# Rayhane-mamah/Tacotron-2

Hardware: NVIDIA H100
Metric: wavenet_train_audio_samples_per_sec (higher is better)
Workload: dtype bf16

## Files before the change

include/t2b200.h:

```cpp
#ifndef T2B200_H_
#define T2B200_H_

#include <stdint.h>

#ifdef __cplusplus
extern "C" {
#endif

#define T2B200_ABI_VERSION 3

#define T2_OK 0
#define T2_ERR_INVALID_ARG (-1)
#define T2_ERR_UNSUPPORTED_SHAPE (-2)
#define T2_ERR_CUDA (-3)
#define T2_ERR_NCCL (-4)

const char* t2_last_error(void);
int t2_abi_version(void);
int t2_struct_size(const char* name);
long long t2_launch_count(void);

int t2_dbg_conv_gemm(const void* d_a, int B, int T, int C, int ld, const int* shifts, int nshift,
                     const void* d_w, int N, int BN, const float* d_bias, int relu, void* d_out_bf16,
                     float* d_out_f32, void* stream);
int t2_dbg_set_timing_buffer(long long* d_buf);
int t2_dbg_wgrad(const void* d_a, int Ca, const void* d_bm, int Cb, int B, int T, int shift_a, float scale,
                 float* d_out, void* stream);

typedef struct {
  const void* ptr;
  int C, T, B, L, ld;
} t2_dbg_act_t;
typedef struct {
  int map, shift, k0, nkb, layer0, nlayers;
} t2_dbg_seg_t;
typedef struct {
  t2_dbg_act_t a[4];
  int na;
  t2_dbg_seg_t seg[16];
  int nseg;
  const void* w;
  int wN, wK, wL, w_layer, w_k0;
  int T, B, n_tiles, ksplit, epi, BN;
  int cluster;
  int cluster_used;
  void* ptr[12];
  float f[6];
  int i[12];
  unsigned long long seed;
} t2_dbg_gemm_t;
int t2_dbg_act_gemm(t2_dbg_gemm_t* call, void* stream);
typedef struct {
  int a_map, a_ch0, a_shift, a_layer;
  int b_map, b_ch0, b_shift, b_layer;
  long long out_off;
  int ldc, m_valid, n_valid;
  float scale;
  int accumulate;
  const float* div;
} t2_dbg_wgrad_tile_t;
int t2_dbg_wgrad_tiles(const t2_dbg_act_t* maps, int nmaps, const t2_dbg_wgrad_tile_t* tiles, int ntiles, float* d_out, int T, int B,
                       void* stream);
int t2_dbg_fx_colsum(const float* d_addends, int nrows, int ncols, float* d_out, void* stream);

typedef struct {
  int kernel;
  void* p[16];
  long long i[16];
  float f[4];
  unsigned long long seed;
  const unsigned long long* step;
} t2_dbg_kernel_t;
#define T2_DBG_TACO_ATT_FWD 1
#define T2_DBG_TACO_BN_FWD 2
#define T2_DBG_TACO_BN_BWD 3
#define T2_DBG_TACO_CELL_BWD 4
#define T2_DBG_TACO_ATT_FINISH 5
#define T2_DBG_TACO_DVALUES 6
#define T2_DBG_TACO_ATT_BWD 7
#define T2_DBG_TACO_CONV_GEMM 8
#define T2_DBG_TACO_LSTM_STEP 9
#define T2_DBG_TACO_ROWS 10
int t2_dbg_taco_kernel(const t2_dbg_kernel_t* call, void* stream);
#define T2_DBG_CBHG_BN_FWD 1
#define T2_DBG_CBHG_BN_BWD 2
#define T2_DBG_CBHG_POOL_FWD 3
#define T2_DBG_CBHG_POOL_BWD 4
#define T2_DBG_CBHG_HIGHWAY_FWD 5
#define T2_DBG_CBHG_HIGHWAY_BWD 6
#define T2_DBG_CBHG_GRU_FWD 7
#define T2_DBG_CBHG_GRU_BWD 8
int t2_dbg_cbhg_kernel(const t2_dbg_kernel_t* call, void* stream);


typedef struct {
  int layers, stacks, residual_channels, gate_channels, skip_out_channels;
  int kernel_size;
  int cin_channels;
  int out_channels;
  int quantize_channels;
  int input_type;
  int legacy, residual_legacy;
  int upsample_type;
  int n_upsample;
  int upsample_scales[4];
  int freq_axis_kernel_size;
  float dropout;
  float log_scale_min;
  int B, T, Tc;
  int c_pre_upsampled;
  float log_scale_min_gauss;
  int cdf_loss;
  int split_bf16;
  int gin_channels;
  int n_speakers;
  int upsample_activation;
  float leaky_alpha;
} t2_wn_config_t;

typedef struct {
  long long n_params;
  long long packed_bytes;
  long long workspace_bytes;
  int n_tensors;
} t2_wn_sizes_t;

int t2_wn_sizes(const t2_wn_config_t* cfg, t2_wn_sizes_t* out);
int t2_wn_param_info(const t2_wn_config_t* cfg, int i, char* name, int name_cap, long long* offset, int* ndim,
                     int* shape4);
int t2_wn_init(const t2_wn_config_t* cfg, void* d_packed, void* d_workspace, void* stream);
int t2_wn_pack_weights(const t2_wn_config_t* cfg, const float* d_params, void* d_packed, void* d_workspace,
                       void* stream);
int t2_wn_forward(const t2_wn_config_t* cfg, const float* d_params, const void* d_packed, void* d_workspace,
                  const void* d_x, const float* d_c, const void* d_targets, const int* d_lengths, float* d_loss,
                  float* d_logits, int save_for_backward, unsigned long long seed,
                  const unsigned long long* d_step, void* stream);
int t2_wn_backward(const t2_wn_config_t* cfg, const float* d_params, const void* d_packed, void* d_workspace,
                   const void* d_x, const float* d_c, float* d_grads, unsigned long long seed,
                   const unsigned long long* d_step, void* stream);
int t2_wn_backward_phased(const t2_wn_config_t* cfg, const float* d_params, const void* d_packed, void* d_workspace,
                          const void* d_x, const float* d_c, float* d_grads, unsigned long long seed,
                          const unsigned long long* d_step, int phase, int n_groups, void* stream);
int t2_wn_time_kernel(const t2_wn_config_t* cfg, const float* d_params, const void* d_packed, void* d_workspace,
                      int which, int layer, int reps, float* ms_per_launch, void* stream);
int t2_dbg_wn_per_layer(int mode);
int t2_dbg_wn_chain(const t2_wn_config_t* cfg, int dir, int* out, int cap);
int t2_wn_workspace_tensor(const t2_wn_config_t* cfg, void* d_workspace, const char* name, void** ptr,
                           long long* count, int* elem_bytes);
int t2_wn_set_speakers(const t2_wn_config_t* cfg, void* d_workspace, const int* d_speaker_ids, void* stream);
#define T2_DBG_WN_UP_FWD 1
#define T2_DBG_WN_UP_BWD_PARAM 2
#define T2_DBG_WN_UP_BWD_INPUT 3
#define T2_DBG_WN_FIRST_CONV 10
#define T2_DBG_WN_FIRST_CONV_BWD 11
#define T2_DBG_WN_COLSUM 12
#define T2_DBG_WN_DERIVED_BIAS 13
#define T2_DBG_WN_SKIP_BIAS 14
#define T2_DBG_WN_FX_FINALIZE 15
#define T2_DBG_WN_CL_TO_CHW 16
#define T2_DBG_WN_GIN_BIAS 17
#define T2_DBG_WN_SET_SPEAKERS 18
#define T2_DBG_WN_GIN_WGRAD 19
#define T2_DBG_WN_GIN_DEMB 20
int t2_dbg_wn_kernel(const t2_dbg_kernel_t* call, void* stream);


int t2_wn_ar_sizes(const t2_wn_config_t* cfg, int cluster_size, long long* packed_bytes, long long* workspace_bytes);
int t2_wn_ar_pack(const t2_wn_config_t* cfg, int cluster_size, const float* d_params, void* d_packed_ar,
                  void* d_workspace, void* stream);
int t2_wn_ar_generate(const t2_wn_config_t* cfg, int cluster_size, const float* d_params, const void* d_packed_ar,
                      void* d_workspace, const float* d_c, const void* d_initial, const void* d_test_inputs,
                      const float* d_u_a, const float* d_u_b, unsigned long long seed, void* d_out_samples,
                      float* d_out_raw, void* stream);
int t2_wn_ar_set_speakers(const t2_wn_config_t* cfg, int cluster_size, const float* d_params, const void* d_packed_ar,
                          void* d_workspace, const int* d_speaker_ids, void* stream);


typedef struct {
  int B, T_in, T_out;
  int n_symbols, num_mels, embedding_dim;
  int enc_conv_layers, enc_conv_kernel, enc_conv_channels, encoder_lstm_units;
  int attention_dim, attention_filters, attention_kernel;
  int prenet1, prenet2, decoder_lstm_units;
  int postnet_layers, postnet_kernel, postnet_channels;
  int clip_outputs;
  float dropout_rate;
  float zoneout_rate;
  float reg_weight;
  float max_abs_value, lower_bound_decay;
  int split_bf16;
  int mask_decoder;
  float cross_entropy_pos_weight;
  int unmasked_encoder;
  int noncumulative_weights;
  float teacher_forcing_ratio;
} t2_taco_config_t;

int t2_taco_sizes(const t2_taco_config_t* cfg, long long* n_params, long long* packed_bytes, long long* workspace_bytes,
                  int* n_tensors);
int t2_taco_param_info(const t2_taco_config_t* cfg, int i, char* name, int name_cap, long long* offset, int* ndim,
                       int* shape4, int* trainable);
int t2_taco_init(const t2_taco_config_t* cfg, void* d_packed, void* d_workspace, void* stream);
int t2_taco_pack_weights(const t2_taco_config_t* cfg, const float* d_params, void* d_packed, void* d_workspace, void* stream);
int t2_taco_forward(const t2_taco_config_t* cfg, float* d_params, const void* d_packed, void* d_workspace,
                    const int* d_inputs, const int* d_input_lengths, const float* d_mel_targets,
                    const float* d_stop_targets, float* d_loss, int training, unsigned long long seed,
                    const unsigned long long* d_step, void* stream);
int t2_taco_set_target_lengths(const t2_taco_config_t* cfg, void* d_workspace, const int* d_target_lengths, void* stream);
int t2_taco_backward(const t2_taco_config_t* cfg, const float* d_params, const void* d_packed, void* d_workspace,
                     const int* d_inputs, const int* d_input_lengths, const float* d_mel_targets,
                     const float* d_stop_targets, float* d_grads, unsigned long long seed,
                     const unsigned long long* d_step, void* stream);
int t2_taco_backward_ex(const t2_taco_config_t* cfg, const float* d_params, const void* d_packed, void* d_workspace,
                     const int* d_inputs, const int* d_input_lengths, const float* d_mel_targets,
                     const float* d_stop_targets, float* d_grads, const float* d_mel_outputs_grad, unsigned long long seed,
                     const unsigned long long* d_step, void* stream);
int t2_taco_infer_begin(const t2_taco_config_t* cfg, float* d_params, const void* d_packed, void* d_workspace,
                        const int* d_inputs, const int* d_input_lengths, void* stream);
int t2_taco_infer_steps(const t2_taco_config_t* cfg, float* d_params, const void* d_packed, void* d_workspace,
                        const int* d_input_lengths, int t_begin, int t_end, unsigned long long seed, void* stream);
int t2_taco_infer_finish(const t2_taco_config_t* cfg, float* d_params, const void* d_packed, void* d_workspace, int T_used,
                         void* stream);
int t2_rng_uniform_f32(unsigned long long seed, unsigned int stream_id, long long first_index, long long n, float* d_out,
                       void* stream);
int t2_dbg_att_stamps(long long* d_buf);
int t2_dbg_ar_stamps(long long* d_buf);
int t2_taco_workspace_tensor(const t2_taco_config_t* cfg, void* d_workspace, const char* name, void** ptr,
                             long long* count, int* elem_bytes);

typedef struct {
  int B, T;
  int num_mels;
  int kernels;
  int conv_channels;
  int pool_size;
  int projection;
  int projection_kernel_size;
  int highwaynet_layers;
  int highway_units;
  int rnn_units;
  int num_freq;
  int n_priority_freq;
  int clip_outputs, mask_decoder;
  float max_abs_value, lower_bound_decay, reg_weight;
  int split_bf16;
} t2_cbhg_config_t;
int t2_cbhg_sizes(const t2_cbhg_config_t* cfg, long long* n_params, long long* packed_bytes, long long* workspace_bytes, int* n_tensors);
int t2_cbhg_param_info(const t2_cbhg_config_t* cfg, int i, char* name, int name_cap, long long* offset, int* ndim, int* shape4,
                       int* trainable);
int t2_cbhg_init(const t2_cbhg_config_t* cfg, void* d_packed, void* d_workspace, void* stream);
int t2_cbhg_pack_weights(const t2_cbhg_config_t* cfg, const float* d_params, void* d_packed, void* d_workspace, void* stream);
int t2_cbhg_set_target_lengths(const t2_cbhg_config_t* cfg, void* d_workspace, const int* d_target_lengths, void* stream);
int t2_cbhg_forward(const t2_cbhg_config_t* cfg, float* d_params, const void* d_packed, void* d_workspace, const float* d_mel,
                    const float* d_linear_targets, float* d_loss, int training, void* stream);
int t2_cbhg_backward(const t2_cbhg_config_t* cfg, const float* d_params, const void* d_packed, void* d_workspace, const float* d_mel,
                     float* d_grads, float* d_mel_grad, void* stream);
int t2_cbhg_workspace_tensor(const t2_cbhg_config_t* cfg, void* d_workspace, const char* name, void** ptr, long long* count);

int t2_adam_step(float* d_params, const float* d_grads, float* d_m, float* d_v, float* d_ema,
                 const long long* d_offsets, int n_tensors, long long n_total, float lr, float beta1, float beta2,
                 float eps, int step, float grad_scale, float max_norm, float max_value, float global_norm_clip,
                 float ema_decay, float* d_scratch, void* stream);

typedef struct {
  int sample_rate, n_fft, hop_size, win_size, num_mels;
  float fmin, fmax;
  float magnitude_power;
  float min_level_db, ref_level_db, max_abs_value;
  int symmetric_mels, allow_clipping_in_normalization, signal_normalization;
} t2_audio_config_t;

int t2_stft_mel_plan_bytes(const t2_audio_config_t* cfg, long long* bytes);
int t2_stft_mel_plan_init(const t2_audio_config_t* cfg, void* d_plan, void* stream);
int t2_stft_mel_frames(const t2_audio_config_t* cfg, int n_samples);
int t2_stft_mel_f32(const t2_audio_config_t* cfg, const void* d_plan, const float* d_wav, int B, int n_samples,
                    float preemphasis, float gain, float* d_mel, float* d_linear, int time_major, void* stream);
int t2_mel_basis_f64(const t2_audio_config_t* cfg, double* h_basis);
int t2_griffin_lim_bytes(const t2_audio_config_t* cfg, int B, int frames, long long* bytes);
int t2_griffin_lim_f32(const t2_audio_config_t* cfg, const void* d_plan, const float* d_mag, float* d_phase_io, int B, int frames,
                       int iters, unsigned long long seed, void* d_workspace, float* d_wav, void* stream);
int t2_preemphasis_f32(const float* d_x, float* d_y, int B, int n_samples, float k, void* stream);
int t2_mulaw_quantize_f32_i32(const float* d_in, int* d_out, long long n, void* stream);
int t2_inv_mulaw_quantize_i32_f32(const int* d_in, float* d_out, long long n, void* stream);
int t2_mulaw_f32(const float* d_in, float* d_out, long long n, void* stream);
int t2_inv_mulaw_f32(const float* d_in, float* d_out, long long n, void* stream);

#ifdef __cplusplus
}
#endif
#endif
```

tacotron-2_b200/csrc/t2_api.cu:

```cuda
#include <stdarg.h>
#include <stdio.h>
#include <stddef.h>
#include <string.h>

#include <vector>

#include "../../include/t2b200.h"
#include "t2_common.cuh"
#include "t2_gemm.h"

#include <atomic>
static thread_local char g_err[512] = "";
static std::atomic<long long> g_launches{0};
void t2_count_launch(int n) { g_launches.fetch_add(n, std::memory_order_relaxed); }
extern "C" long long t2_launch_count(void) { return g_launches.load(std::memory_order_relaxed); }

int t2_set_error(int code, const char* fmt, ...) {
  va_list ap;
  va_start(ap, fmt);
  vsnprintf(g_err, sizeof(g_err), fmt, ap);
  va_end(ap);
  return code;
}

extern "C" const char* t2_last_error(void) { return g_err; }
extern "C" int t2_abi_version(void) { return T2B200_ABI_VERSION; }

extern "C" int t2_dbg_conv_gemm(const void* a, int B, int T, int C, int ld, const int* shifts, int nshift,
                                const void* w, int N, int BN, const float* bias, int relu, void* out_bf16,
                                float* out_f32, void* stream) {
  using namespace t2;
  T2_REQUIRE(nshift >= 1 && nshift <= kMaxSeg, T2_ERR_INVALID_ARG, "nshift out of range");
  T2_REQUIRE(BN == 128 || BN == 256, T2_ERR_UNSUPPORTED_SHAPE, "BN must be 128 or 256");
  ActGemmCall c;
  memset(&c, 0, sizeof(c));
  c.a[0] = make_act(a, C, T, B, 1, ld);
  c.na = 1;
  const int nkb = (C + kBK - 1) / kBK;
  for (int s = 0; s < nshift; ++s) c.seg[s] = Seg{0, shifts[s], 0, nkb, 0, 1};
  c.nseg = nshift;
  c.w = w; c.wN = N; c.wK = nshift * nkb * kBK; c.wL = 1; c.w_layer = 0;
  c.T = T; c.B = B; c.n_tiles = (N + BN - 1) / BN;
  c.epi.ptr[0] = out_bf16; c.epi.ptr[1] = const_cast<float*>(bias); c.epi.ptr[2] = out_f32;
  c.epi.i[0] = N; c.epi.i[1] = relu; c.epi.i[2] = N;
  return launch_act_gemm(EPI_BIAS_ACT, BN, c, static_cast<cudaStream_t>(stream));
}

extern "C" int t2_dbg_wgrad(const void* a, int Ca, const void* bm, int Cb, int B, int T, int shift_a,
                            float scale, float* out, void* stream) {
  using namespace t2;
  ActT maps[2] = {make_act(a, Ca, T, B), make_act(bm, Cb, T, B)};
  WgradTile proto;
  memset(&proto, 0, sizeof(proto));
  proto.a_map = 0; proto.a_shift = shift_a; proto.b_map = 1; proto.scale = scale;
  std::vector<WgradTile> tiles;
  append_wgrad_tiles(tiles, proto, 0, Ca, 0, Cb, 0, Cb);
  WgradTile* dt = nullptr;
  cudaStream_t st = static_cast<cudaStream_t>(stream);
  T2_CHECK_CUDA(cudaMallocAsync(&dt, tiles.size() * sizeof(WgradTile), st));
  T2_CHECK_CUDA(cudaMemcpyAsync(dt, tiles.data(), tiles.size() * sizeof(WgradTile), cudaMemcpyHostToDevice, st));
  int rc = launch_wgrad(maps, 2, dt, int(tiles.size()), out, T, B, st);
  cudaStreamSynchronize(st);
  cudaFreeAsync(dt, st);
  return rc;
}

#define T2_SAME_FIELD(A, B, f) static_assert(offsetof(A, f) == offsetof(B, f), #A " / " #B ": field " #f)
static_assert(sizeof(t2_dbg_act_t) == sizeof(t2::ActT), "t2_dbg_act_t / ActT");
T2_SAME_FIELD(t2_dbg_act_t, t2::ActT, ptr); T2_SAME_FIELD(t2_dbg_act_t, t2::ActT, C); T2_SAME_FIELD(t2_dbg_act_t, t2::ActT, ld);
static_assert(sizeof(t2_dbg_seg_t) == sizeof(t2::Seg), "t2_dbg_seg_t / Seg");
T2_SAME_FIELD(t2_dbg_seg_t, t2::Seg, map); T2_SAME_FIELD(t2_dbg_seg_t, t2::Seg, nlayers);
static_assert(sizeof(t2_dbg_wgrad_tile_t) == sizeof(t2::WgradTile), "t2_dbg_wgrad_tile_t / WgradTile");
T2_SAME_FIELD(t2_dbg_wgrad_tile_t, t2::WgradTile, a_map); T2_SAME_FIELD(t2_dbg_wgrad_tile_t, t2::WgradTile, a_ch0);
T2_SAME_FIELD(t2_dbg_wgrad_tile_t, t2::WgradTile, a_shift); T2_SAME_FIELD(t2_dbg_wgrad_tile_t, t2::WgradTile, a_layer);
T2_SAME_FIELD(t2_dbg_wgrad_tile_t, t2::WgradTile, b_map); T2_SAME_FIELD(t2_dbg_wgrad_tile_t, t2::WgradTile, b_ch0);
T2_SAME_FIELD(t2_dbg_wgrad_tile_t, t2::WgradTile, b_shift); T2_SAME_FIELD(t2_dbg_wgrad_tile_t, t2::WgradTile, b_layer);
T2_SAME_FIELD(t2_dbg_wgrad_tile_t, t2::WgradTile, out_off); T2_SAME_FIELD(t2_dbg_wgrad_tile_t, t2::WgradTile, ldc);
T2_SAME_FIELD(t2_dbg_wgrad_tile_t, t2::WgradTile, m_valid); T2_SAME_FIELD(t2_dbg_wgrad_tile_t, t2::WgradTile, n_valid);
T2_SAME_FIELD(t2_dbg_wgrad_tile_t, t2::WgradTile, scale); T2_SAME_FIELD(t2_dbg_wgrad_tile_t, t2::WgradTile, accumulate);
T2_SAME_FIELD(t2_dbg_wgrad_tile_t, t2::WgradTile, div);
#undef T2_SAME_FIELD

extern "C" int t2_dbg_act_gemm(t2_dbg_gemm_t* call, void* stream) {
  using namespace t2;
  T2_REQUIRE(call != nullptr, T2_ERR_INVALID_ARG, "null call");
  T2_REQUIRE(call->na >= 1 && call->na <= 4 && call->nseg >= 1 && call->nseg <= kMaxSeg, T2_ERR_INVALID_ARG,
             "bad map/segment count (%d, %d)", call->na, call->nseg);
  ActGemmCall c;
  memset(&c, 0, sizeof(c));
  memcpy(c.a, call->a, sizeof(c.a));
  c.na = call->na;
  memcpy(c.seg, call->seg, sizeof(c.seg));
  c.nseg = call->nseg;
  c.w = call->w; c.wN = call->wN; c.wK = call->wK; c.wL = call->wL; c.w_layer = call->w_layer; c.w_k0 = call->w_k0;
  c.T = call->T; c.B = call->B; c.n_tiles = call->n_tiles; c.ksplit = call->ksplit; c.cluster = call->cluster;
  memcpy(c.epi.ptr, call->ptr, sizeof(c.epi.ptr));
  memcpy(c.epi.f, call->f, sizeof(c.epi.f));
  memcpy(c.epi.i, call->i, sizeof(c.epi.i));
  c.epi.seed = call->seed;
  call->cluster_used = 0;
  return launch_act_gemm(call->epi, call->BN, c, static_cast<cudaStream_t>(stream), &call->cluster_used);
}

extern "C" int t2_dbg_wgrad_tiles(const t2_dbg_act_t* maps, int nmaps, const t2_dbg_wgrad_tile_t* tiles, int ntiles, float* d_out, int T,
                                  int B, void* stream) {
  using namespace t2;
  T2_REQUIRE(maps && tiles && nmaps >= 1 && nmaps <= 6 && ntiles >= 1, T2_ERR_INVALID_ARG, "wgrad_tiles: bad map/tile arguments");
  for (int i = 0; i < ntiles; ++i)
    T2_REQUIRE(tiles[i].a_map >= 0 && tiles[i].a_map < nmaps && tiles[i].b_map >= 0 && tiles[i].b_map < nmaps &&
               tiles[i].m_valid >= 1 && tiles[i].m_valid <= 128 && tiles[i].n_valid >= 1 && tiles[i].n_valid <= 256 &&
               tiles[i].accumulate >= 0 && tiles[i].accumulate <= 2,
               T2_ERR_INVALID_ARG, "wgrad_tiles: bad tile %d", i);
  WgradTile* dt = nullptr;
  cudaStream_t st = static_cast<cudaStream_t>(stream);
  T2_CHECK_CUDA(cudaMallocAsync(&dt, ntiles * sizeof(WgradTile), st));
  const cudaError_t e = cudaMemcpyAsync(dt, tiles, ntiles * sizeof(WgradTile), cudaMemcpyHostToDevice, st);
  int rc = e == cudaSuccess ? launch_wgrad(reinterpret_cast<const ActT*>(maps), nmaps, dt, ntiles, d_out, T, B, st)
                            : t2_set_error(T2_ERR_CUDA, "wgrad_tiles: tile table upload failed: %s", cudaGetErrorString(e));
  cudaStreamSynchronize(st);
  cudaFreeAsync(dt, st);
  return rc;
}

__global__ void fx_colsum_kernel(const float* __restrict__ v, long long n, int ncols, long long* acc) {
  const long long i = blockIdx.x * (long long)blockDim.x + threadIdx.x;
  if (i < n) t2::fx_add(acc + i % ncols, v[i]);
}
extern "C" int t2_dbg_fx_colsum(const float* d_addends, int nrows, int ncols, float* d_out, void* stream) {
  T2_REQUIRE(d_addends && d_out && nrows >= 0 && ncols >= 1, T2_ERR_INVALID_ARG, "fx_colsum: bad arguments");
  cudaStream_t st = static_cast<cudaStream_t>(stream);
  long long* acc = nullptr;
  T2_CHECK_CUDA(cudaMallocAsync(&acc, size_t(ncols) * sizeof(long long), st));
  const long long n = (long long)nrows * ncols;
  cudaError_t e = cudaMemsetAsync(acc, 0, size_t(ncols) * sizeof(long long), st);
  if (e == cudaSuccess) e = cudaMemsetAsync(d_out, 0, size_t(ncols) * sizeof(float), st);
  if (e == cudaSuccess && n > 0) {
    fx_colsum_kernel<<<unsigned((n + 255) / 256), 256, 0, st>>>(d_addends, n, ncols, acc);
    t2_count_launch();
    e = cudaGetLastError();
  }
  int rc = e == cudaSuccess ? t2::launch_fx_finalize(acc, d_out, ncols, st)
                            : t2_set_error(T2_ERR_CUDA, "fx_colsum: %s", cudaGetErrorString(e));
  cudaStreamSynchronize(st);
  cudaFreeAsync(acc, st);
  return rc;
}

extern "C" int t2_dbg_set_timing_buffer(long long* d_buf) {
  t2::set_timing_buffer(d_buf);
  return T2_OK;
}

__global__ void rng_uniform_kernel(unsigned long long seed, unsigned int stream, long long i0, long long n, float* __restrict__ out) {
  const long long i = blockIdx.x * (long long)blockDim.x + threadIdx.x;
  if (i < n) out[i] = t2::hash_uniform32(t2::hash_seed(seed, stream), (unsigned long long)(i0 + i));
}
extern "C" int t2_rng_uniform_f32(unsigned long long seed, unsigned int stream_id, long long first_index, long long n, float* d_out,
                                  void* stream) {
  T2_REQUIRE(n >= 0 && (n == 0 || d_out != nullptr), T2_ERR_INVALID_ARG, "rng_uniform: bad arguments");
  if (n == 0) return T2_OK;
  rng_uniform_kernel<<<unsigned((n + 255) / 256), 256, 0, static_cast<cudaStream_t>(stream)>>>(seed, stream_id, first_index, n, d_out);
  t2_count_launch();
  T2_CHECK_CUDA(cudaGetLastError());
  return T2_OK;
}

extern "C" int t2_struct_size(const char* name) {
  if (!name) return -1;
  if (!strcmp(name, "t2_wn_config_t")) return int(sizeof(t2_wn_config_t));
  if (!strcmp(name, "t2_wn_sizes_t")) return int(sizeof(t2_wn_sizes_t));
  if (!strcmp(name, "t2_taco_config_t")) return int(sizeof(t2_taco_config_t));
  if (!strcmp(name, "t2_cbhg_config_t")) return int(sizeof(t2_cbhg_config_t));
  if (!strcmp(name, "t2_audio_config_t")) return int(sizeof(t2_audio_config_t));
  if (!strcmp(name, "t2_dbg_act_t")) return int(sizeof(t2_dbg_act_t));
  if (!strcmp(name, "t2_dbg_gemm_t")) return int(sizeof(t2_dbg_gemm_t));
  if (!strcmp(name, "t2_dbg_wgrad_tile_t")) return int(sizeof(t2_dbg_wgrad_tile_t));
  if (!strcmp(name, "t2_dbg_kernel_t")) return int(sizeof(t2_dbg_kernel_t));
  return -1;
}
```

tacotron-2_b200/csrc/t2_cbhg.cu:

```cuda
#include <math.h>
#include <stdio.h>
#include <string.h>

#include <string>
#include <vector>

#include "../../include/t2b200.h"
#include "t2_batchnorm.h"
#include "t2_common.cuh"
#include "t2_gemm.h"
#include "t2_params.h"

namespace t2 {
namespace {

typedef __nv_bfloat16 bf16;
constexpr int kMaxBank = 16, kMaxHw = 8;
constexpr int kGruItems = 4;
constexpr int kGruThreads = 256;

struct CConv {
  int cin, cout, k, act;
  ConvBnParams p;
  int cinp, coutp;
// ... 493 lines not shown
      for (int q = 0; q < 2; ++q) {
        const float2 v = *reinterpret_cast<const float2*>(dcp + (2 * half + q) * kRU + 2 * jp);
        drh[q] += v.x * w0 + v.y * w1;
      }
    }
#pragma unroll
    for (int q = 0; q < 2; ++q) {
      const int i = 2 * half + q;
      const long long row = (long long)(b0 + i) * a.T + t;
      const float drp = drh[q] * hp[q] * rv[q] * (1.f - rv[q]);
      const float dup = du[q] * uv[q] * (1.f - uv[q]);
      dgp[i * 2 * kRU + k2] = drp; dgp[i * 2 * kRU + kRU + k2] = dup;
      if (b0 + i < a.B) {
        a.dXP[row * XPW + d * 3 * kRU + k2] = __float2bfloat16(drp);
        a.dXP[row * XPW + d * 3 * kRU + kRU + k2] = __float2bfloat16(dup);
      }
      part[q] += drh[q] * rv[q];
    }
    __syncthreads();
#pragma unroll 4
    for (int jp = 0; jp < 128; ++jp) {
      const uint32_t w = WgT[jp * 128 + k2];
      const float w0 = bf16lo(w), w1 = bf16hi(w);
#pragma unroll
      for (int q = 0; q < 2; ++q) {
        const float2 v = *reinterpret_cast<const float2*>(dgp + (2 * half + q) * 2 * kRU + 2 * jp);
        part[q] += v.x * w0 + v.y * w1;
      }
    }
#pragma unroll
    for (int q = 0; q < 2; ++q) dh[(2 * half + q) * kRU + k2] = part[q];
    __syncthreads();
  }
}

int gemm(const void* a, int C, int ld, int k0, long long T, int Bn, const void* w, int wN, int wK, int ntaps, const int* shifts, int BN,
         const float* bias, int act, void* out_bf16, float* out_f32, int ldo, int nvalid, cudaStream_t st, const int* k0s = nullptr, int Ctot = 0,
         int split = 0) {
  ActGemmCall g;
  memset(&g, 0, sizeof(g));
  if (split) {
    const int rc = set_split_operand(g, a, C, int(T), Bn, ntaps, shifts);
    if (rc) return rc;
  } else {
    const int nkb = (C + kBK - 1) / kBK;
    g.a[0] = make_act(a, Ctot > 0 ? Ctot : k0 + C, int(T), Bn, 1, ld); g.na = 1;
    T2_REQUIRE(ntaps <= kMaxSeg, T2_ERR_UNSUPPORTED_SHAPE, "CBHG gemm: too many taps");
    for (int s = 0; s < ntaps; ++s) g.seg[s] = Seg{0, shifts ? shifts[s] : 0, k0s ? k0s[s] : k0, nkb, 0, 1};
    g.nseg = ntaps;
  }
  g.w = w; g.wN = wN; g.wK = wK; g.wL = 1;
  g.T = int(T); g.B = Bn; g.n_tiles = (nvalid + BN - 1) / BN;
  g.epi.ptr[0] = out_bf16; g.epi.ptr[1] = const_cast<float*>(bias); g.epi.ptr[2] = out_f32;
  g.epi.i[0] = ldo; g.epi.i[1] = act; g.epi.i[2] = nvalid;
  return launch_act_gemm(EPI_BIAS_ACT, BN, g, st);
}

enum { WG_LIN = 0, WG_GRU = 1, WG_HW0 = 2  };
void build_tiles(const CL& lo, std::vector<std::vector<WgradTile>>& L) {
  L.clear();
  const int RU = lo.RU, HU = lo.HU;
  { std::vector<WgradTile> w; append_wgrad_tiles(w, dense_proto(0, 1), 0, 2 * RU, 0, lo.NF, lo.p_lk, lo.NF); L.push_back(w); }
  { std::vector<WgradTile> w;
    for (int d = 0; d < 2; ++d) {
      append_wgrad_tiles(w, dense_proto(0, 1), 0, HU, d * 3 * RU, 2 * RU, lo.p_gk[d], 2 * RU);
      append_wgrad_tiles(w, dense_proto(0, 1), 0, HU, d * 3 * RU + 2 * RU, RU, lo.p_ck[d], RU);
      append_wgrad_tiles(w, dense_proto(2, 1, d == 0 ? -1 : 1), d * RU, RU, d * 3 * RU, 2 * RU, lo.p_gk[d] + (long long)HU * 2 * RU, 2 * RU);
      append_wgrad_tiles(w, dense_proto(3 + d, 1), 0, RU, d * 3 * RU + 2 * RU, RU, lo.p_ck[d] + (long long)HU * RU, RU);
    }
    L.push_back(w); }
  for (int i = lo.NH - 1; i >= 0; --i) {
    std::vector<WgradTile> w;
    append_wgrad_tiles(w, dense_proto(0, 1), 0, HU, 0, HU, lo.p_hk[i][0], HU);
    append_wgrad_tiles(w, dense_proto(0, 1), 0, HU, HU, HU, lo.p_hk[i][1], HU);
    L.push_back(w);
  }
  { std::vector<WgradTile> w; append_wgrad_tiles(w, dense_proto(0, 1), 0, lo.M, 0, HU, lo.p_dk, HU); L.push_back(w); }
  for (const CConv* c : {&lo.proj2, &lo.proj1}) {
    std::vector<WgradTile> w; append_conv_wgrad_tiles(w, c->k, 0, c->cin, 0, c->cout, c->p.kernel); L.push_back(w);
  }
  { std::vector<WgradTile> w;
    for (int k = 1; k <= lo.K; ++k) append_conv_wgrad_tiles(w, k, 0, lo.M, (k - 1) * lo.CC, lo.CC, lo.bank[k - 1].p.kernel);
    L.push_back(w); }
}

size_t gru_fwd_smem(int split) { return (64 * 256 + 64 * 128) * 4 * (split ? 2 : 1) + 3 * kGruItems * kRU * 4; }
size_t gru_bwd_smem() { return (128 * 128 + 64 * 128) * 4 + (2 * kGruItems * kRU + kGruItems * 2 * kRU) * 4; }

int gru_setup() {
  T2_CHECK_CUDA(cudaFuncSetAttribute(gru_fwd_kernel<false>, cudaFuncAttributeMaxDynamicSharedMemorySize, int(gru_fwd_smem(0))));
  T2_CHECK_CUDA(cudaFuncSetAttribute(gru_fwd_kernel<true>, cudaFuncAttributeMaxDynamicSharedMemorySize, int(gru_fwd_smem(1))));
  T2_CHECK_CUDA(cudaFuncSetAttribute(gru_bwd_kernel, cudaFuncAttributeMaxDynamicSharedMemorySize, int(gru_bwd_smem())));
  return T2_OK;
}
int check_gru_shape(int B, int T, int HU, int RU, const char* what) {
  T2_REQUIRE(B >= 1 && T >= 1 && HU >= 1, T2_ERR_UNSUPPORTED_SHAPE, "%s: B >= 1, T >= 1, HU >= 1 (B %d, T %d, HU %d)", what, B, T, HU);
  T2_REQUIRE(RU == kRU, T2_ERR_UNSUPPORTED_SHAPE, "%s: RU must be %d (got %d)", what, kRU, RU);
  return T2_OK;
}
int check_gru_fwd(const GruArgs& a, int split) {
  T2_REQUIRE(a.params && a.XP && a.out, T2_ERR_INVALID_ARG, "gru_fwd: null params / XP / out");
  T2_REQUIRE(split == 0 || split == 1, T2_ERR_INVALID_ARG, "gru_fwd: split %d is not 0 or 1", split);
  int n = 0;
  for (int d = 0; d < 2; ++d) n += (a.r[d] != nullptr) + (a.u[d] != nullptr) + (a.c[d] != nullptr) + (a.rh[d] != nullptr);
  T2_REQUIRE(!split || n == 0, T2_ERR_INVALID_ARG, "gru_fwd: the split mode writes no stashes (%d of 8 given)", n);
  T2_REQUIRE(n == 0 || n == 8, T2_ERR_INVALID_ARG, "gru_fwd: the r / u / c / rh stashes of both directions are all present or all null (%d of 8)", n);
  for (int d = 0; d < 2; ++d)
    T2_REQUIRE(a.p_gk[d] >= 0 && a.p_ck[d] >= 0 && a.p_gb[d] >= 0 && a.p_cb[d] >= 0, T2_ERR_INVALID_ARG, "gru_fwd: negative parameter offset");
  return check_gru_shape(a.B, a.T, a.HU, a.RU, "gru_fwd");
}
int check_gru_bwd(const GruBwdArgs& a) {
  T2_REQUIRE(a.params && a.dout && a.out && a.dXP, T2_ERR_INVALID_ARG, "gru_bwd: null params / dout / out / dXP");
  for (int d = 0; d < 2; ++d) {
    T2_REQUIRE(a.r[d] && a.u[d] && a.c[d], T2_ERR_INVALID_ARG, "gru_bwd: null stash of direction %d", d);
    T2_REQUIRE(a.p_gk[d] >= 0 && a.p_ck[d] >= 0, T2_ERR_INVALID_ARG, "gru_bwd: negative parameter offset");
  }
  return check_gru_shape(a.B, a.T, a.HU, a.RU, "gru_bwd");
}
int launch_gru_fwd(const GruArgs& a, int split, cudaStream_t st) {
  int rc = check_gru_fwd(a, split);
  if (rc) return rc;
  (split ? gru_fwd_kernel<true> : gru_fwd_kernel<false>)<<<dim3((a.B + kGruItems - 1) / kGruItems, 2), kGruThreads, gru_fwd_smem(split), st>>>(a);
  t2_count_launch();
  T2_CHECK_CUDA(cudaGetLastError());
  return T2_OK;
}
int launch_gru_bwd(const GruBwdArgs& a, cudaStream_t st) {
  int rc = check_gru_bwd(a);
  if (rc) return rc;
  gru_bwd_kernel<<<dim3((a.B + kGruItems - 1) / kGruItems, 2), kGruThreads, gru_bwd_smem(), st>>>(a); t2_count_launch();
  T2_CHECK_CUDA(cudaGetLastError());
  return T2_OK;
}

}
}

using namespace t2;

extern "C" int t2_cbhg_sizes(const t2_cbhg_config_t* cfg, long long* n_params, long long* packed_bytes, long long* workspace_bytes, int* n_tensors) {
  CL lo;
  int rc = build(cfg, lo, nullptr);
  if (rc) return rc;
  if (n_params) *n_params = lo.n_params;
  if (packed_bytes) *packed_bytes = lo.packed_bytes;
  if (workspace_bytes) *workspace_bytes = lo.workspace_bytes;
  if (n_tensors) *n_tensors = int(lo.params.size());
  return T2_OK;
}

extern "C" int t2_cbhg_param_info(const t2_cbhg_config_t* cfg, int i, char* name, int cap, long long* offset, int* ndim, int* shape4, int* trainable) {
  CL lo;
  int rc = build(cfg, lo, nullptr);
  if (rc) return rc;
  return param_info(lo.params, i, name, cap, offset, ndim, shape4, trainable);
}

extern "C" int t2_cbhg_init(const t2_cbhg_config_t* cfg, void* d_packed, void* d_workspace, void* stream) {
  CL lo;
  std::vector<PackJob> jobs;
  int rc = build(cfg, lo, &jobs);
  if (rc) return rc;
  T2_REQUIRE(d_packed && d_workspace, T2_ERR_INVALID_ARG, "cbhg_init: null buffers");
  cudaStream_t st = static_cast<cudaStream_t>(stream);
  uint8_t* ws = static_cast<uint8_t*>(d_workspace);
  T2_CHECK_CUDA(cudaMemsetAsync(d_packed, 0, lo.packed_bytes, st));
  T2_CHECK_CUDA(cudaMemsetAsync(d_workspace, 0, lo.workspace_bytes, st));
  T2_CHECK_CUDA(cudaMemcpyAsync(ws + lo.w_jobs, jobs.data(), jobs.size() * sizeof(PackJob), cudaMemcpyHostToDevice, st));
  std::vector<std::vector<WgradTile>> wl;
  build_tiles(lo, wl);
  std::vector<WgradTile> all;
  for (auto& w : wl) all.insert(all.end(), w.begin(), w.end());
  T2_REQUIRE(all.size() <= 4096, T2_ERR_UNSUPPORTED_SHAPE, "cbhg: too many wgrad tiles (%d)", int(all.size()));
  T2_CHECK_CUDA(cudaMemcpyAsync(ws + lo.w_tiles, all.data(), all.size() * sizeof(WgradTile), cudaMemcpyHostToDevice, st));
  rc = upload_reg_table(lo.params, ws + lo.w_regtab, st);
  if (rc) return rc;
  rc = gru_setup();
  if (rc) return rc;
  T2_CHECK_CUDA(cudaStreamSynchronize(st));
  return T2_OK;
}

extern "C" int t2_cbhg_pack_weights(const t2_cbhg_config_t* cfg, const float* d_params, void* d_packed, void* d_workspace, void* stream) {
  CL lo;
  int rc = build(cfg, lo, nullptr);
  if (rc) return rc;
  return launch_pack(d_params, d_packed, reinterpret_cast<const PackJob*>(static_cast<uint8_t*>(d_workspace) + lo.w_jobs), lo.n_jobs, 32, 32,
                     static_cast<cudaStream_t>(stream));
}

extern "C" int t2_cbhg_set_target_lengths(const t2_cbhg_config_t* cfg, void* d_workspace, const int* d_target_lengths, void* stream) {
  CL lo;
  int rc = build(cfg, lo, nullptr);
  if (rc) return rc;
  T2_REQUIRE(d_workspace && d_target_lengths, T2_ERR_INVALID_ARG, "cbhg_set_target_lengths: null pointer");
  T2_CHECK_CUDA(cudaMemcpyAsync(static_cast<uint8_t*>(d_workspace) + lo.w_tlen, d_target_lengths, lo.B * sizeof(int), cudaMemcpyDeviceToDevice,
                                static_cast<cudaStream_t>(stream)));
  return T2_OK;
}

namespace {
struct Ctx { const CL* lo; uint8_t* ws; const uint8_t* pk; float* params; cudaStream_t st; int training; };
template <typename T> T* W(const Ctx& s, long long off) { return reinterpret_cast<T*>(s.ws + off); }

int conv_fwd(const Ctx& s, const CConv& L, const void* x, int ld_x, bf16* y_b, float* y_f, int ldo) {
  int shifts[16];
  for (int j = 0; j < L.k; ++j) shifts[j] = conv_tap_shift(L.k, j);
  const int BN = L.cout % 256 == 0 ? 256 : 128;
  const int sp = s.lo->c.split_bf16;
  return gemm(x, L.cin, ld_x, 0, s.lo->T, s.lo->B, s.pk + L.k_w, (L.cout + 127) / 128 * 128, L.k * L.cinp * (sp ? 3 : 1), L.k, shifts, BN,
              s.params + L.p.bias, L.act, y_b, y_f, ldo, L.cout, s.st, nullptr, 0, sp);
}
}

extern "C" int t2_cbhg_forward(const t2_cbhg_config_t* cfg, float* d_params, const void* d_packed, void* d_workspace, const float* d_mel,
                               const float* d_linear_targets, float* d_loss, int training, void* stream) {
  CL lo;
  int rc = build(cfg, lo, nullptr);
  if (rc) return rc;
  T2_REQUIRE(d_params && d_packed && d_workspace && d_mel, T2_ERR_INVALID_ARG, "cbhg_forward: null pointer");
  cudaStream_t st = static_cast<cudaStream_t>(stream);
  Ctx s{&lo, static_cast<uint8_t*>(d_workspace), static_cast<const uint8_t*>(d_packed), d_params, st, training};
  const long long N = lo.N;
  const int T = lo.T, B = lo.B, M = lo.M, HU = lo.HU, RU = lo.RU, KC = lo.KC, PJc = lo.PJc;
  float* scal = W<float>(s, lo.w_scal);
  T2_CHECK_CUDA(cudaMemsetAsync(scal, 0, 16 * sizeof(float), st));
  const int sp = lo.c.split_bf16, k3 = sp ? 3 : 1, Ms = (M + 63) / 64 * 64;
  bf16* x0 = W<bf16>(s, lo.w_x0);
  if (sp) launch_f32_to_bf16_split(d_mel, x0, N, M, Ms, st);
  else launch_f32_to_bf16(d_mel, x0, N * M, st);
  bf16* Y = W<bf16>(s, lo.w_Y);
  float* Yf = W<float>(s, lo.w_Y);
  bf16* Xb = W<bf16>(s, lo.w_Xb);
  float* stb = W<float>(s, lo.w_stb);
  if (training) T2_CHECK_CUDA(cudaMemsetAsync(stb, 0, 2LL * KC * sizeof(float), st));
  for (int k = 1; k <= lo.K; ++k) {
    const CConv& L = lo.bank[k - 1];
    const int c0 = (k - 1) * lo.CC;
// ... 331 lines not shown
```

tacotron-2_b200/csrc/t2_common.cuh:

```cuda
#pragma once
#include <cuda.h>
#include <cuda_bf16.h>
#include <cuda_runtime.h>
#include <stdint.h>

#define T2_OK 0
#define T2_ERR_INVALID_ARG (-1)
#define T2_ERR_UNSUPPORTED_SHAPE (-2)
#define T2_ERR_CUDA (-3)
#define T2_ERR_NCCL (-4)

int t2_set_error(int code, const char* fmt, ...);
void t2_count_launch(int n = 1);
#define T2_CHECK_CUDA(expr)                                                              \
  do {                                                                                   \
    cudaError_t _e = (expr);                                                             \
    if (_e != cudaSuccess)                                                               \
      return t2_set_error(T2_ERR_CUDA, "%s:%d %s -> %s", __FILE__, __LINE__, #expr,      \
                          cudaGetErrorString(_e));                                       \
  } while (0)
#define T2_REQUIRE(cond, code, ...)                                                      \
  do {                                                                                   \
    if (!(cond)) return t2_set_error(code, __VA_ARGS__);                                 \
  } while (0)
// ... 103 lines not shown
  if (fx_in_range(v)) {
    x.a = v;
    x.old = static_cast<long long>(atomicAdd(x.d, static_cast<unsigned long long>(v)));
  }
  return x;
}
__device__ __forceinline__ void fx_check(const FxAdd& x) {
  if (!fx_in_range(x.old) || !fx_in_range(x.old + x.a)) atomicExch(x.d, static_cast<unsigned long long>(kFxPoison));
}
__device__ __forceinline__ void fx_add(long long* dst, float v) { fx_check(fx_issue(dst, v)); }
__device__ __forceinline__ float fx_value(long long a) {
  return fx_in_range(a) ? float(double(a) * (1.0 / 1099511627776.0)) : __int_as_float(0x7fffffff);
}
int launch_fx_finalize(const long long* acc, float* out, long long n, cudaStream_t st);

__device__ __forceinline__ void mbar_init(uint64_t* bar, uint32_t count) {
  asm volatile("mbarrier.init.shared::cta.b64 [%0], %1;\n" ::"r"(smem_u32(bar)), "r"(count));
}
__device__ __forceinline__ void fence_barrier_init() {
  asm volatile("fence.mbarrier_init.release.cluster;\n" ::: "memory");
}
__device__ __forceinline__ void fence_proxy_async() {
  asm volatile("fence.proxy.async.shared::cta;\n" ::: "memory");
}
__device__ __forceinline__ void mbar_expect_tx(uint64_t* bar, uint32_t bytes) {
  asm volatile("mbarrier.arrive.expect_tx.shared::cta.b64 _, [%0], %1;\n" ::"r"(smem_u32(bar)),
               "r"(bytes)
               : "memory");
}
__device__ __forceinline__ void mbar_arrive(uint64_t* bar) {
  asm volatile("mbarrier.arrive.shared::cta.b64 _, [%0];\n" ::"r"(smem_u32(bar)) : "memory");
}
__device__ __forceinline__ bool mbar_try_wait(uint64_t* bar, uint32_t parity) {
  uint32_t ok;
  asm volatile(
      "{\n\t.reg .pred P;\n\t"
      "mbarrier.try_wait.parity.shared::cta.b64 P, [%1], %2;\n\t"
      "selp.u32 %0, 1, 0, P;\n\t}\n"
      : "=r"(ok)
      : "r"(smem_u32(bar)), "r"(parity)
      : "memory");
  return ok != 0;
}
__device__ __forceinline__ void mbar_wait(uint64_t* bar, uint32_t parity) {
  while (!mbar_try_wait(bar, parity)) {
  }
}

__device__ __forceinline__ void tma_prefetch_desc(const CUtensorMap* m) {
  asm volatile("prefetch.tensormap [%0];\n" ::"l"(reinterpret_cast<uint64_t>(m)) : "memory");
}
__device__ __forceinline__ void tma_load_2d(void* smem, const CUtensorMap* m, uint64_t* bar, int c0,
                                            int c1) {
  asm volatile(
      "cp.async.bulk.tensor.2d.shared::cluster.global.tile.mbarrier::complete_tx::bytes "
      "[%0], [%1, {%3, %4}], [%2];\n" ::"r"(smem_u32(smem)),
      "l"(reinterpret_cast<uint64_t>(m)), "r"(smem_u32(bar)), "r"(c0), "r"(c1)
      : "memory");
}
__device__ __forceinline__ void tma_load_3d(void* smem, const CUtensorMap* m, uint64_t* bar, int c0,
                                            int c1, int c2) {
  asm volatile(
      "cp.async.bulk.tensor.3d.shared::cluster.global.tile.mbarrier::complete_tx::bytes "
      "[%0], [%1, {%3, %4, %5}], [%2];\n" ::"r"(smem_u32(smem)),
      "l"(reinterpret_cast<uint64_t>(m)), "r"(smem_u32(bar)), "r"(c0), "r"(c1), "r"(c2)
      : "memory");
}
__device__ __forceinline__ void tma_load_4d(void* smem, const CUtensorMap* m, uint64_t* bar, int c0,
                                            int c1, int c2, int c3) {
  asm volatile(
      "cp.async.bulk.tensor.4d.shared::cluster.global.tile.mbarrier::complete_tx::bytes "
      "[%0], [%1, {%3, %4, %5, %6}], [%2];\n" ::"r"(smem_u32(smem)),
      "l"(reinterpret_cast<uint64_t>(m)), "r"(smem_u32(bar)), "r"(c0), "r"(c1), "r"(c2), "r"(c3)
      : "memory");
}

__device__ __forceinline__ void tma_load_3d_mc(void* smem, const CUtensorMap* m, uint64_t* bar, int c0, int c1, int c2, uint16_t cta_mask) {
  asm volatile(
      "cp.async.bulk.tensor.3d.shared::cluster.global.tile.mbarrier::complete_tx::bytes.multicast::cluster "
      "[%0], [%1, {%3, %4, %5}], [%2], %6;\n" ::"r"(smem_u32(smem)),
      "l"(reinterpret_cast<uint64_t>(m)), "r"(smem_u32(bar)), "r"(c0), "r"(c1), "r"(c2), "h"(cta_mask)
      : "memory");
}
__device__ __forceinline__ void tma_store_3d(const CUtensorMap* m, const void* smem, int c0, int c1, int c2) {
  asm volatile("cp.async.bulk.tensor.3d.global.shared::cta.bulk_group [%0, {%2, %3, %4}], [%1];\n" ::"l"(reinterpret_cast<uint64_t>(m)),
               "r"(smem_u32(smem)), "r"(c0), "r"(c1), "r"(c2)
               : "memory");
}
__device__ __forceinline__ void bulk_commit() { asm volatile("cp.async.bulk.commit_group;\n" ::: "memory"); }
template <int N>
__device__ __forceinline__ void bulk_wait_read() { asm volatile("cp.async.bulk.wait_group.read %0;\n" ::"n"(N) : "memory"); }
__device__ __forceinline__ void bulk_wait_all() { asm volatile("cp.async.bulk.wait_group 0;\n" ::: "memory"); }
__device__ __forceinline__ void fence_proxy_async_smem() { asm volatile("fence.proxy.async.shared::cta;\n" ::: "memory"); }
__device__ __forceinline__ uint32_t mapa_cluster(const void* ptr, uint32_t rank) {
  uint32_t r;
  asm volatile("mapa.shared::cluster.u32 %0, %1, %2;" : "=r"(r) : "r"(smem_u32(ptr)), "r"(rank));
  return r;
}
__device__ __forceinline__ uint32_t cluster_ctarank() {
  uint32_t r;
  asm volatile("mov.u32 %0, %%cluster_ctarank;" : "=r"(r));
  return r;
}
__device__ __forceinline__ uint32_t cluster_nctarank() {
  uint32_t r;
  asm volatile("mov.u32 %0, %%cluster_nctarank;" : "=r"(r));
  return r;
}
__device__ __forceinline__ void cluster_sync_all() {
  asm volatile("barrier.cluster.arrive.release.aligned;\n" ::: "memory");
  asm volatile("barrier.cluster.wait.acquire.aligned;\n" ::: "memory");
}
__device__ __forceinline__ void mbar_arrive_cluster(uint64_t* bar, uint32_t rank) {
  asm volatile("mbarrier.arrive.release.cluster.shared::cluster.b64 _, [%0];\n" ::"r"(mapa_cluster(bar, rank)) : "memory");
}

__device__ __forceinline__ void bulk_load_1d(void* smem_dst, const void* gmem_src, uint32_t bytes, uint64_t* bar) {
  asm volatile("cp.async.bulk.shared::cluster.global.mbarrier::complete_tx::bytes [%0], [%1], %2, [%3];\n" ::"r"(smem_u32(smem_dst)),
               "l"(gmem_src), "r"(bytes), "r"(smem_u32(bar))
               : "memory");
}

__device__ __forceinline__ void pdl_wait() { asm volatile("griddepcontrol.wait;" ::: "memory"); }
__device__ __forceinline__ void pdl_launch_dependents() { asm volatile("griddepcontrol.launch_dependents;" ::: "memory"); }

__device__ __forceinline__ void wgmma_fence() { asm volatile("wgmma.fence.sync.aligned;\n" ::: "memory"); }
__device__ __forceinline__ void wgmma_commit() { asm volatile("wgmma.commit_group.sync.aligned;\n" ::: "memory"); }
template <int N>
__device__ __forceinline__ void wgmma_wait() { asm volatile("wgmma.wait_group.sync.aligned %0;\n" ::"n"(N) : "memory"); }
template <int R>
__device__ __forceinline__ void wgmma_fence_regs(float (&d)[R]) {
#pragma unroll
  for (int i = 0; i < R; ++i) asm volatile("" : "+f"(d[i])::"memory");
}
template <int N, int TA, int TB> struct Wgmma;
template <int TA, int TB>
struct Wgmma<16, TA, TB> {
  static __device__ __forceinline__ void mma(float (&d)[8], uint64_t da, uint64_t db, uint32_t scale_d) {
    asm volatile(
        "{\n.reg .pred p;\nsetp.ne.b32 p, %10, 0;\n"
        "wgmma.mma_async.sync.aligned.m64n16k16.f32.bf16.bf16 {"
        "%0, %1, %2, %3, %4, %5, %6, %7"
        "}, %8, %9, p, 1, 1, %11, %12;\n}\n"
        : "+f"(d[0]), "+f"(d[1]), "+f"(d[2]), "+f"(d[3]), "+f"(d[4]), "+f"(d[5]), "+f"(d[6]), "+f"(d[7])
        : "l"(da), "l"(db), "r"(scale_d), "n"(TA), "n"(TB));
  }
};
template <int TA, int TB>
struct Wgmma<64, TA, TB> {
  static __device__ __forceinline__ void mma(float (&d)[32], uint64_t da, uint64_t db, uint32_t scale_d) {
    asm volatile(
        "{\n.reg .pred p;\nsetp.ne.b32 p, %34, 0;\n"
        "wgmma.mma_async.sync.aligned.m64n64k16.f32.bf16.bf16 {"
        "%0, %1, %2, %3, %4, %5, %6, %7, %8, %9, %10, %11, %12, %13, %14, %15, "
        "%16, %17, %18, %19, %20, %21, %22, %23, %24, %25, %26, %27, %28, %29, %30, %31"
        "}, %32, %33, p, 1, 1, %35, %36;\n}\n"
        : "+f"(d[0]), "+f"(d[1]), "+f"(d[2]), "+f"(d[3]), "+f"(d[4]), "+f"(d[5]), "+f"(d[6]), "+f"(d[7]),
          "+f"(d[8]), "+f"(d[9]), "+f"(d[10]), "+f"(d[11]), "+f"(d[12]), "+f"(d[13]), "+f"(d[14]), "+f"(d[15]),
          "+f"(d[16]), "+f"(d[17]), "+f"(d[18]), "+f"(d[19]), "+f"(d[20]), "+f"(d[21]), "+f"(d[22]), "+f"(d[23]),
          "+f"(d[24]), "+f"(d[25]), "+f"(d[26]), "+f"(d[27]), "+f"(d[28]), "+f"(d[29]), "+f"(d[30]), "+f"(d[31])
        : "l"(da), "l"(db), "r"(scale_d), "n"(TA), "n"(TB));
  }
};
template <int TA, int TB>
struct Wgmma<128, TA, TB> {
  static __device__ __forceinline__ void mma(float (&d)[64], uint64_t da, uint64_t db, uint32_t scale_d) {
    asm volatile(
        "{\n.reg .pred p;\nsetp.ne.b32 p, %66, 0;\n"
        "wgmma.mma_async.sync.aligned.m64n128k16.f32.bf16.bf16 {"
        "%0, %1, %2, %3, %4, %5, %6, %7, %8, %9, %10, %11, %12, %13, %14, %15, "
        "%16, %17, %18, %19, %20, %21, %22, %23, %24, %25, %26, %27, %28, %29, %30, %31, "
        "%32, %33, %34, %35, %36, %37, %38, %39, %40, %41, %42, %43, %44, %45, %46, %47, "
        "%48, %49, %50, %51, %52, %53, %54, %55, %56, %57, %58, %59, %60, %61, %62, %63"
        "}, %64, %65, p, 1, 1, %67, %68;\n}\n"
        : "+f"(d[0]), "+f"(d[1]), "+f"(d[2]), "+f"(d[3]), "+f"(d[4]), "+f"(d[5]), "+f"(d[6]), "+f"(d[7]),
          "+f"(d[8]), "+f"(d[9]), "+f"(d[10]), "+f"(d[11]), "+f"(d[12]), "+f"(d[13]), "+f"(d[14]), "+f"(d[15]),
          "+f"(d[16]), "+f"(d[17]), "+f"(d[18]), "+f"(d[19]), "+f"(d[20]), "+f"(d[21]), "+f"(d[22]), "+f"(d[23]),
          "+f"(d[24]), "+f"(d[25]), "+f"(d[26]), "+f"(d[27]), "+f"(d[28]), "+f"(d[29]), "+f"(d[30]), "+f"(d[31]),
          "+f"(d[32]), "+f"(d[33]), "+f"(d[34]), "+f"(d[35]), "+f"(d[36]), "+f"(d[37]), "+f"(d[38]), "+f"(d[39]),
          "+f"(d[40]), "+f"(d[41]), "+f"(d[42]), "+f"(d[43]), "+f"(d[44]), "+f"(d[45]), "+f"(d[46]), "+f"(d[47]),
          "+f"(d[48]), "+f"(d[49]), "+f"(d[50]), "+f"(d[51]), "+f"(d[52]), "+f"(d[53]), "+f"(d[54]), "+f"(d[55]),
          "+f"(d[56]), "+f"(d[57]), "+f"(d[58]), "+f"(d[59]), "+f"(d[60]), "+f"(d[61]), "+f"(d[62]), "+f"(d[63])
        : "l"(da), "l"(db), "r"(scale_d), "n"(TA), "n"(TB));
  }
};
template <int TA, int TB>
struct Wgmma<192, TA, TB> {
  static __device__ __forceinline__ void mma(float (&d)[96], uint64_t da, uint64_t db, uint32_t scale_d) {
    asm volatile(
        "{\n.reg .pred p;\nsetp.ne.b32 p, %98, 0;\n"
        "wgmma.mma_async.sync.aligned.m64n192k16.f32.bf16.bf16 {"
        "%0, %1, %2, %3, %4, %5, %6, %7, %8, %9, %10, %11, %12, %13, %14, %15, "
        "%16, %17, %18, %19, %20, %21, %22, %23, %24, %25, %26, %27, %28, %29, %30, %31, "
        "%32, %33, %34, %35, %36, %37, %38, %39, %40, %41, %42, %43, %44, %45, %46, %47, "
        "%48, %49, %50, %51, %52, %53, %54, %55, %56, %57, %58, %59, %60, %61, %62, %63, "
        "%64, %65, %66, %67, %68, %69, %70, %71, %72, %73, %74, %75, %76, %77, %78, %79, "
        "%80, %81, %82, %83, %84, %85, %86, %87, %88, %89, %90, %91, %92, %93, %94, %95"
// ... 62 lines not shown
```

tacotron-2_b200/csrc/t2_gemm.cu:

```cuda
#include <stdlib.h>
#include <mutex>

#include "t2_gemm.cuh"
#include "t2_gemm.h"

namespace t2 {

static long long* g_timing_buffer = nullptr;
void set_timing_buffer(long long* p) { g_timing_buffer = p; }

typedef CUresult (*EncodeTiledFn)(CUtensorMap*, CUtensorMapDataType, cuuint32_t, void*, const cuuint64_t*,
                                  const cuuint64_t*, const cuuint32_t*, const cuuint32_t*,
                                  CUtensorMapInterleave, CUtensorMapSwizzle, CUtensorMapL2promotion,
                                  CUtensorMapFloatOOBfill);

static EncodeTiledFn get_encode_fn() {
  static EncodeTiledFn fn = nullptr;
  static std::once_flag once;
  std::call_once(once, [] {
    void* p = nullptr;
    cudaDriverEntryPointQueryResult q;
    if (cudaGetDriverEntryPoint("cuTensorMapEncodeTiled", &p, cudaEnableDefault, &q) == cudaSuccess &&
        q == cudaDriverEntryPointSuccess)
      fn = reinterpret_cast<EncodeTiledFn>(p);
// ... 135 lines not shown
               "act_gemm: split-K needs atomic accumulation (mode 2) into every destination in use (modes %d, %d)", c.epi.i[2],
               c.epi.i[5]);
  }
  memset(&g, 0, sizeof(g));
  for (int i = 0; i < 4; ++i) {
    int rc = encode_act_map(&g.amap[i], c.a[i < c.na ? i : 0], kBM);
    if (rc) return rc;
  }
  grid = dim3((c.T + kBM - 1) / kBM * c.B, c.n_tiles, c.ksplit > 1 ? c.ksplit : 1);
  cs = pick_cluster(BN, grid, c.cluster);
  int rc = encode_wt_map(&g.bmap, c.w, c.wN, c.wK, c.wL, BN / cs);
  if (rc) return rc;
  for (int s = 0; s < c.nseg; ++s) g.seg[s] = c.seg[s];
  g.nseg = c.nseg;
  g.T = c.T;
  g.tiles_per_b = (c.T + kBM - 1) / kBM;
  g.b_layer = c.w_layer;
  g.b_k0 = c.w_k0;
  g.dbg = g_timing_buffer;
  g.epi = c.epi;
  if (!c.epi.i[11]) {
    const void* outs[3] = {nullptr, nullptr, nullptr};
    int ldo = 0;
    if (epi == EPI_GATE) { outs[0] = c.epi.ptr[0]; outs[1] = c.epi.ptr[1]; outs[2] = c.epi.ptr[2]; ldo = c.epi.i[0]; }
    else if (epi == EPI_RES) { outs[0] = c.epi.ptr[1]; outs[1] = c.epi.ptr[2]; ldo = BN; }
    else if (epi == EPI_GATE_BWD) { outs[0] = c.epi.ptr[2]; ldo = 2 * c.epi.i[0]; }
    else if (epi == EPI_DX) { outs[0] = c.epi.ptr[1]; ldo = BN; }
    for (int i = 0; i < 3; ++i)
      if (outs[i]) {
        rc = encode_out_map(&g.omap[i], outs[i], ldo, c.T, c.B);
        if (rc) return rc;
      }
  }
  return T2_OK;
}

long long* take_timing_slice(long long n_slots) {
  long long* p = g_timing_buffer;
  if (p) g_timing_buffer = p + n_slots;
  return p;
}

int set_split_operand(ActGemmCall& c, const void* a, int C, int T, int B, int ntaps, const int* shifts) {
  const int nkb = (C + kBK - 1) / kBK, Cp = nkb * kBK;
  T2_REQUIRE(2 * ntaps <= kMaxSeg, T2_ERR_UNSUPPORTED_SHAPE, "split-bf16 GEMM: %d taps are more than %d segments", ntaps, kMaxSeg);
  c.a[0] = make_act(a, 2 * Cp, T, B, 1, 2 * Cp); c.na = 1;
  c.nseg = 0;
  for (int s = 0; s < ntaps; ++s) {
    c.seg[c.nseg++] = Seg{0, shifts ? shifts[s] : 0, 0, 2 * nkb, 0, 1};
    c.seg[c.nseg++] = Seg{0, shifts ? shifts[s] : 0, 0, nkb, 0, 1};
  }
  c.epi.i[11] = 1;
  return T2_OK;
}

int launch_act_gemm(int epi, int BN, const ActGemmCall& c, cudaStream_t stream, int* cluster_used) {
  GemmArgs g;
  dim3 grid;
  int cs = 1;
  const int rc = make_gemm_args(epi, BN, c, g, grid, cs);
  if (rc) return rc;
  if (cluster_used) *cluster_used = cs;
#define T2_CASE(E, N) \
  if (epi == E && BN == N) return launch_one<E, N>(g, grid, cs, stream);
  T2_CASE(EPI_GATE, 256)
  T2_CASE(EPI_RES, 128)
  T2_CASE(EPI_RES, 256)
  T2_CASE(EPI_BIAS_ACT, 128)
  T2_CASE(EPI_BIAS_ACT, 256)
  T2_CASE(EPI_CE, 256)
  T2_CASE(EPI_SCALE_RELUMASK, 128)
  T2_CASE(EPI_SCALE_RELUMASK, 256)
  T2_CASE(EPI_GATE_BWD, 128)
  T2_CASE(EPI_GATE_BWD, 256)
  T2_CASE(EPI_DX, 128)
  T2_CASE(EPI_DX, 256)
  T2_CASE(EPI_MOL, 32)
  T2_CASE(EPI_LSTM, 32)
  T2_CASE(EPI_TOUT, 32)
#undef T2_CASE
  return t2_set_error(T2_ERR_UNSUPPORTED_SHAPE, "act_gemm: no kernel for epilogue %d with BN=%d", epi, BN);
}

int launch_wgrad(const ActT* maps, int nmaps, const WgradTile* tiles_dev, int ntiles, float* out, int T,
                 int B, cudaStream_t stream) {
  T2_REQUIRE(nmaps >= 1 && nmaps <= 6 && ntiles >= 1, T2_ERR_INVALID_ARG, "wgrad: bad map/tile count");
  WgradArgs g;
  memset(&g, 0, sizeof(g));
  for (int i = 0; i < 6; ++i) {
    int rc = encode_act_map(&g.map[i], maps[i < nmaps ? i : 0], kBK);
    if (rc) return rc;
  }
  g.tiles = tiles_dev;
  g.out = out;
  g.T = T;
  g.B = B;
  static bool configured = false;
  if (!configured) {
    T2_CHECK_CUDA(cudaFuncSetAttribute(wgrad_gemm_kernel, cudaFuncAttributeMaxDynamicSharedMemorySize, kWgSmemBytes));
    configured = true;
  }
  cudaLaunchConfig_t cfg;
  memset(&cfg, 0, sizeof(cfg));
  cfg.gridDim = dim3(ntiles); cfg.blockDim = dim3(kGemmThreads); cfg.dynamicSmemBytes = kWgSmemBytes; cfg.stream = stream;
  cudaLaunchAttribute attr[1];
  attr[0].id = cudaLaunchAttributeProgrammaticStreamSerialization;
  attr[0].val.programmaticStreamSerializationAllowed = 1;
  cfg.attrs = attr; cfg.numAttrs = pdl_enabled() ? 1 : 0;
  T2_CHECK_CUDA(cudaLaunchKernelEx(&cfg, wgrad_gemm_kernel, g));
  t2_count_launch();
  return T2_OK;
}

void append_wgrad_tiles(std::vector<WgradTile>& v, const WgradTile& proto, int a_ch0, int Ca, int b_ch0, int Cb, long long out_off,
                        int ldc) {
  for (int m0 = 0; m0 < Ca; m0 += kWgBM)
    for (int n0 = 0; n0 < Cb; n0 += kWgBN) {
      WgradTile t;
      memset(&t, 0, sizeof(t));
      t.a_map = proto.a_map; t.a_ch0 = a_ch0 + m0; t.a_shift = proto.a_shift; t.a_layer = proto.a_layer;
      t.b_map = proto.b_map; t.b_ch0 = b_ch0 + n0; t.b_shift = proto.b_shift; t.b_layer = proto.b_layer;
      t.out_off = out_off + (long long)m0 * ldc + n0; t.ldc = ldc;
      t.m_valid = Ca - m0 < kWgBM ? Ca - m0 : kWgBM;
      t.n_valid = Cb - n0 < kWgBN ? Cb - n0 : kWgBN;
      t.scale = proto.scale; t.accumulate = proto.accumulate; t.div = proto.div;
      v.push_back(t);
    }
}

WgradTile dense_proto(int am, int bm, int a_shift) {
  WgradTile t;
  memset(&t, 0, sizeof(t));
  t.a_map = am; t.a_shift = a_shift; t.b_map = bm; t.scale = 1.f;
  return t;
}

void append_conv_wgrad_tiles(std::vector<WgradTile>& v, int k, int a_ch0, int Ca, int b_ch0, int Cb, long long out_off) {
  for (int j = 0; j < k; ++j)
    append_wgrad_tiles(v, dense_proto(0, 1, conv_tap_shift(k, j)), a_ch0, Ca, b_ch0, Cb, out_off + (long long)j * Ca * Cb, Cb);
}

constexpr long long kChainTimeoutNs = 1000000000LL;

__device__ __forceinline__ int ld_acquire_gpu(const int* p) {
  int v;
  asm volatile("ld.acquire.gpu.global.b32 %0, [%1];" : "=r"(v) : "l"(p) : "memory");
  return v;
}
__device__ __forceinline__ void red_release_gpu_add(int* p, int v) {
  asm volatile("red.release.gpu.global.add.s32 [%0], %1;" ::"l"(p), "r"(v) : "memory");
}
__device__ __forceinline__ void fence_proxy_async_global() { asm volatile("fence.proxy.async.global;" ::: "memory"); }

template <int BN>
__device__ __forceinline__ void chain_inval_barriers(uint8_t* smem) {
  using Cfg = ActGemmCfg<BN>;
  uint64_t* full_bar = Cfg::full_bar(smem);
  for (int i = 0; i < 2 * Cfg::kStages; ++i)
    asm volatile("mbarrier.inval.shared::cta.b64 [%0];" ::"r"(smem_u32(&full_bar[i])) : "memory");
}

template <bool FWD, int BN0, int BN1>
__global__ void __launch_bounds__(kActGemmThreads, 1) wn_chain_kernel(const __grid_constant__ ChainArgs a) {
  constexpr int E0 = FWD ? EPI_GATE : EPI_GATE_BWD, E1 = FWD ? EPI_RES : EPI_DX;
  using C0 = ActGemmCfg<BN0>;
  using C1 = ActGemmCfg<BN1>;
  static_assert(C0::kPipeBytes == C1::kPipeBytes && C0::kEpiBytes == C1::kEpiBytes && C0::kSmemBytes == C1::kSmemBytes,
                "both GEMMs of a chain share one shared-memory plan");
  extern __shared__ uint8_t smem_raw[];
  uint8_t* smem = reinterpret_cast<uint8_t*>((reinterpret_cast<uintptr_t>(smem_raw) + 1023) & ~uintptr_t(1023));
  __shared__ EpiArgs s_epi;
  __shared__ int s_ticket;
  int* done = a.ctr + 16;
  int* stop = a.ctr + 1;
  int prev_kind = -1;
  for (;;) {
    if (threadIdx.x == 0) {
      int t = atomicAdd(a.ctr, 1);
      if (t < a.n_tix && *reinterpret_cast<volatile int*>(stop) == 0) {
        long long* dbg = a.dbg ? a.dbg + size_t(t) * kDbgSlots : nullptr;
        const long long t_start = globaltimer_ns();
        if (dbg) { dbg[0] = t_start; dbg[3] = smid(); }
        const ChainTicket k = a.tix[t];
        for (int i = k.dep_lo; i <= k.dep_hi && t < a.n_tix; ++i)
          while (ld_acquire_gpu(done + i) < k.dep_target) {
            if (globaltimer_ns() - t_start > kChainTimeoutNs) {
              if (atomicExch(stop, 1) == 0) atomicAdd(a.err, 1);
              t = a.n_tix;
              break;
            }
            __nanosleep(32);
          }
        fence_proxy_async_global();
        if (dbg) dbg[1] = globaltimer_ns();
// ... 62 lines not shown
```

tacotron-2_b200/csrc/t2_gemm.cuh:

```cuda
#pragma once
#include "t2_common.cuh"
#include "t2_gemm_types.h"

namespace t2 {

__device__ __forceinline__ void store_bf16x32(__nv_bfloat16* dst, const float (&v)[32]) {
  uint4* d = reinterpret_cast<uint4*>(dst);
#pragma unroll
  for (int q = 0; q < 4; ++q) {
    uint4 u;
    u.x = pack_bf16x2(v[q * 8 + 0], v[q * 8 + 1]);
    u.y = pack_bf16x2(v[q * 8 + 2], v[q * 8 + 3]);
    u.z = pack_bf16x2(v[q * 8 + 4], v[q * 8 + 5]);
    u.w = pack_bf16x2(v[q * 8 + 6], v[q * 8 + 7]);
    d[q] = u;
  }
}
__device__ __forceinline__ void load_bf16x32(const __nv_bfloat16* src, float (&v)[32]) {
  const uint4* s = reinterpret_cast<const uint4*>(src);
#pragma unroll
  for (int q = 0; q < 4; ++q) {
    uint4 u = __ldg(s + q);
    v[q * 8 + 0] = bf16lo(u.x); v[q * 8 + 1] = bf16hi(u.x);
    v[q * 8 + 2] = bf16lo(u.y); v[q * 8 + 3] = bf16hi(u.y);
// ... 973 lines not shown
      wgmma_fence_regs(d);
#pragma unroll
      for (int k = 0; k < kBK / 16; ++k)
        Wgmma<WN, 0, 0>::mma(d, adesc + uint64_t(k * 2), bdesc + uint64_t(k * 2), (kb > 0 || k > 0) ? 1u : 0u);
      wgmma_commit();
      wgmma_fence_regs(d);
      wgmma_wait<1>();
      if (kb > 0 && lane == 0) {
        if (cs == 1) mbar_arrive(&empty_bar[prev]);
        else for (uint32_t r = 0; r < cs; ++r) mbar_arrive_cluster(&empty_bar[prev], r);
      }
      prev = stage;
      if (++stage == Cfg::kStages) { stage = 0; phase ^= 1; }
    }
    wgmma_wait<0>();
    wgmma_fence_regs(d);
    if (dbg && threadIdx.x == 0) dbg[3] = clock64();
    asm volatile("bar.sync 6, 512;\n" ::: "memory");
    {
      const int r0 = mh * 64 + (warp & 3) * 16 + (lane >> 2);
#pragma unroll
      for (int j = 0; j < WN / 8; ++j)
#pragma unroll
        for (int i = 0; i < 2; ++i) {
          const int r = r0 + 8 * i, col = nh * WN + 8 * j + 2 * (lane & 3);
          *reinterpret_cast<float2*>(acc_s + r * BN + ((((col >> 2) ^ (r & 7)) << 2) | (col & 3))) =
              make_float2(d[4 * j + 2 * i], d[4 * j + 2 * i + 1]);
        }
    }
    asm volatile("bar.sync 6, 512;\n" ::: "memory");
    const int row = q * 32 + lane;
    c.trow = AccRow{acc_s + row * BN, 0, row & 7};
    if (dbg && threadIdx.x == 0) dbg[4] = clock64();
    if constexpr (kCoh) Epilogue<EPI, BN>::template run<kChain>(epi, c);
    else Epilogue<EPI, BN>::run(epi, c);
    if (dbg && threadIdx.x == 0) dbg[5] = clock64();
    tile_store_drain(c);
  }
}

template <int EPI, int BN>
__global__ void __launch_bounds__(kActGemmThreads, 1) act_gemm_kernel(const __grid_constant__ GemmArgs g) {
  using Cfg = ActGemmCfg<BN>;
  extern __shared__ uint8_t smem_raw[];
  uint8_t* smem = reinterpret_cast<uint8_t*>((reinterpret_cast<uintptr_t>(smem_raw) + 1023) & ~uintptr_t(1023));
  const int m_tile = blockIdx.x;
  const int b = m_tile / g.tiles_per_b;
  const int t0 = (m_tile - b * g.tiles_per_b) * kBM;
  int all_kb = 0;
  for (int s = 0; s < g.nseg; ++s) all_kb += g.seg[s].nkb * g.seg[s].nlayers;
  const int kb_lo = int((long long)all_kb * blockIdx.z / gridDim.z), kb_hi = int((long long)all_kb * (blockIdx.z + 1) / gridDim.z);

  const uint32_t cs = cluster_nctarank(), crank = cluster_ctarank();
  const uint16_t cmask = uint16_t((1u << cs) - 1u);
  long long* dbg = g.dbg ? g.dbg + ((size_t(blockIdx.z) * gridDim.y + blockIdx.y) * gridDim.x + blockIdx.x) * kDbgSlots : nullptr;
  if (dbg && threadIdx.x == 0) { dbg[0] = clock64(); dbg[8] = globaltimer_ns(); dbg[11] = smid(); }

  if ((threadIdx.x >> 5) == kActEpiWarps && elect_one()) {
    for (int i = 0; i < 4; ++i) tma_prefetch_desc(&g.amap[i]);
    tma_prefetch_desc(&g.bmap);
    Cfg::init_barriers(smem, kActEpiWarps * cs);
  }
  __syncthreads();
  if (cs > 1) cluster_sync_all();
  pdl_wait();
  pdl_launch_dependents();
  if (dbg && threadIdx.x == 0) { dbg[1] = clock64(); dbg[9] = globaltimer_ns(); }

  act_gemm_tile<EPI, BN>(g, g.epi, smem, m_tile, blockIdx.y, b, t0, kb_lo, kb_hi, cs, crank, cmask, dbg);
  __syncthreads();
  if (dbg && threadIdx.x == 0) { dbg[6] = clock64(); dbg[10] = globaltimer_ns(); }
  if (cs > 1) cluster_sync_all();
}

constexpr int kWgBM = 128;
constexpr int kWgBN = 256;
constexpr int kWgStages = 4;
constexpr int kWgStageBytes = 6 * (kBK * 128);
constexpr int kWgSmemBytes = kWgStages * kWgStageBytes + 1024 + 256;
static_assert(kWgSmemBytes <= 232448, "shared memory budget");

template <int N>
__device__ __forceinline__ void wgrad_consume(const WgradArgs& g, const WgradTile& tile, uint8_t* smem, uint64_t* full_bar,
                                              uint64_t* empty_bar, int total_kb) {
  constexpr int kBlk = kBK * 128;
  const int warp = threadIdx.x >> 5, lane = threadIdx.x & 31, wg = warp >> 2;
  float d[N / 2];
#pragma unroll
  for (int i = 0; i < N / 2; ++i) d[i] = 0.f;
  int stage = 0, prev = 0;
  uint32_t phase = 0;
  for (int kb = 0; kb < total_kb; ++kb) {
    mbar_wait(&full_bar[stage], phase);
    __syncwarp();
    const uint32_t sa = smem_u32(smem + stage * kWgStageBytes) + uint32_t(wg * kBlk);
    const uint32_t sb = smem_u32(smem + stage * kWgStageBytes + 2 * kBlk);
    const uint64_t adesc = make_gdesc_sw128(sa, kBlk, 1024);
    const uint64_t bdesc = make_gdesc_sw128(sb, kBlk, 1024);
    wgmma_fence();
    wgmma_fence_regs(d);
#pragma unroll
    for (int k = 0; k < kBK / 16; ++k)
      Wgmma<N, 1, 1>::mma(d, adesc + uint64_t(k * 128), bdesc + uint64_t(k * 128), (kb > 0 || k > 0) ? 1u : 0u);
    wgmma_commit();
    wgmma_fence_regs(d);
    wgmma_wait<1>();
    if (kb > 0 && lane == 0) mbar_arrive(&empty_bar[prev]);
    prev = stage;
    if (++stage == kWgStages) { stage = 0; phase ^= 1; }
  }
  wgmma_wait<0>();
  wgmma_fence_regs(d);
  float sc = tile.scale;
  if (tile.div) sc /= fmaxf(__ldg(tile.div), 1e-20f);
  float* out = g.out + tile.out_off;
  const int m0 = wg * 64 + (warp & 3) * 16 + (lane >> 2);
#pragma unroll
  for (int j = 0; j < N / 8; ++j)
#pragma unroll
    for (int i = 0; i < 2; ++i)
#pragma unroll
      for (int e = 0; e < 2; ++e) {
        const int m = m0 + 8 * i, n = 8 * j + 2 * (lane & 3) + e;
        if (m < tile.m_valid && n < tile.n_valid) {
          float* o = out + size_t(m) * tile.ldc + n;
          const float r = d[4 * j + 2 * i + e] * sc;
          if (tile.accumulate == 2) atomicAdd(o, r);
          else if (tile.accumulate == 1) *o += r;
          else *o = r;
        }
      }
}

__global__ void __launch_bounds__(kGemmThreads, 1) wgrad_gemm_kernel(const __grid_constant__ WgradArgs g) {
  extern __shared__ uint8_t smem_raw[];
  uint8_t* smem = reinterpret_cast<uint8_t*>((reinterpret_cast<uintptr_t>(smem_raw) + 1023) & ~uintptr_t(1023));
  uint64_t* full_bar = reinterpret_cast<uint64_t*>(smem + kWgStages * kWgStageBytes);
  uint64_t* empty_bar = full_bar + kWgStages;
  const int warp = threadIdx.x >> 5;
  const WgradTile tile = g.tiles[blockIdx.x];
  const int kb_per_b = (g.T + kBK - 1) / kBK;
  const int total_kb = kb_per_b * g.B;
  const int nblk = (tile.n_valid + 63) >> 6;

  if (warp == 8 && elect_one()) {
    for (int i = 0; i < kWgStages; ++i) { mbar_init(&full_bar[i], 1); mbar_init(&empty_bar[i], 8); }
    fence_barrier_init();
  }
  __syncthreads();
  pdl_wait();
  pdl_launch_dependents();
  constexpr int kBlk = kBK * 128;

  if (warp == 8) {
    if (elect_one()) {
      int stage = 0; uint32_t phase = 0;
      for (int bb = 0; bb < g.B; ++bb)
        for (int kb = 0; kb < kb_per_b; ++kb) {
          mbar_wait(&empty_bar[stage], phase ^ 1);
          mbar_expect_tx(&full_bar[stage], uint32_t(2 + nblk) * kBlk);
          uint8_t* sa = smem + stage * kWgStageBytes;
          uint8_t* sb = sa + 2 * kBlk;
          const int tpos = kb * kBK;
          tma_load_4d(sa, &g.map[tile.a_map], &full_bar[stage], tile.a_ch0, tpos + tile.a_shift, bb, tile.a_layer);
          tma_load_4d(sa + kBlk, &g.map[tile.a_map], &full_bar[stage], tile.a_ch0 + 64, tpos + tile.a_shift, bb, tile.a_layer);
          for (int i = 0; i < nblk; ++i)
            tma_load_4d(sb + i * kBlk, &g.map[tile.b_map], &full_bar[stage], tile.b_ch0 + 64 * i, tpos + tile.b_shift, bb, tile.b_layer);
          if (++stage == kWgStages) { stage = 0; phase ^= 1; }
        }
    }
  } else {
    switch (nblk) {
      case 1: wgrad_consume<64>(g, tile, smem, full_bar, empty_bar, total_kb); break;
      case 2: wgrad_consume<128>(g, tile, smem, full_bar, empty_bar, total_kb); break;
      case 3: wgrad_consume<192>(g, tile, smem, full_bar, empty_bar, total_kb); break;
      default: wgrad_consume<256>(g, tile, smem, full_bar, empty_bar, total_kb); break;
    }
  }
}

}
```

tacotron-2_b200/csrc/t2_gemm.h:

```cpp
#pragma once
#include <cuda_runtime.h>
#include <string.h>

#include <vector>

#include "t2_gemm_types.h"

namespace t2 {

struct ActT {
  const void* ptr;
  int C, T, B, L, ld;
};
inline ActT make_act(const void* p, int C, int T, int B, int L = 1, int ld = -1) {
  ActT a;
  a.ptr = p; a.C = C; a.T = T; a.B = B; a.L = L; a.ld = ld < 0 ? C : ld;
  return a;
}

struct ActGemmCall {
  ActT a[4];
  int na;
  Seg seg[kMaxSeg];
  int nseg;
  const void* w;
  int wN, wK, wL, w_layer, w_k0;
  int T, B;
  int n_tiles;
  int ksplit;
  int cluster;
  EpiArgs epi;
};

void set_timing_buffer(long long* p);
bool pdl_enabled();
int cluster_pref();
template <typename... KArgs, typename... Args>
inline cudaError_t launch_pdl(void (*kernel)(KArgs...), dim3 grid, dim3 block, size_t smem, cudaStream_t st, Args... args) {
  cudaLaunchConfig_t cfg;
  memset(&cfg, 0, sizeof(cfg));
  cfg.gridDim = grid; cfg.blockDim = block; cfg.dynamicSmemBytes = smem; cfg.stream = st;
  cudaLaunchAttribute attr[1];
  attr[0].id = cudaLaunchAttributeProgrammaticStreamSerialization;
  attr[0].val.programmaticStreamSerializationAllowed = 1;
  cfg.attrs = attr; cfg.numAttrs = pdl_enabled() ? 1 : 0;
  return cudaLaunchKernelEx(&cfg, kernel, KArgs(args)...);
}
int set_split_operand(ActGemmCall& c, const void* a, int C, int T, int B, int ntaps, const int* shifts);
int launch_act_gemm(int epi, int BN, const ActGemmCall& c, cudaStream_t stream, int* cluster_used = nullptr);
int make_gemm_args(int epi, int BN, const ActGemmCall& c, GemmArgs& g, dim3& grid, int& cs);
int launch_wn_chain(bool fwd, int bn0, int bn1, const ChainArgs& a, int grid, cudaStream_t st);
long long* take_timing_slice(long long n_slots);
int launch_wgrad(const ActT* maps, int nmaps, const WgradTile* tiles_dev, int ntiles, float* out,
                 int T, int B, cudaStream_t stream);
void append_wgrad_tiles(std::vector<WgradTile>& v, const WgradTile& proto, int a_ch0, int Ca, int b_ch0, int Cb, long long out_off,
                        int ldc);
WgradTile dense_proto(int am, int bm, int a_shift = 0);
inline int conv_tap_shift(int k, int j) { return j - (k - 1) / 2; }
void append_conv_wgrad_tiles(std::vector<WgradTile>& v, int k, int a_ch0, int Ca, int b_ch0, int Cb, long long out_off);

}
```

tacotron-2_b200/csrc/t2_gemm_types.h:

```cpp
#pragma once
#include <cuda.h>
#include <stdint.h>

namespace t2 {

constexpr int kBM = 128;
constexpr int kBK = 64;
constexpr int kMaxSeg = 16;
constexpr int kGemmThreads = 288;
constexpr int kDbgSlots = 16;

struct Seg {
  int map;
  int shift;
  int k0;
  int nkb;
  int layer0;
  int nlayers;
};

struct EpiArgs {
  void* ptr[12];
  float f[6];
  int i[12];
  unsigned long long seed;
};

struct GemmArgs {
  CUtensorMap amap[4];
  CUtensorMap bmap;
  CUtensorMap omap[3];
  Seg seg[kMaxSeg];
  int nseg;
  int T;
  int tiles_per_b;
  int b_layer;
  int b_k0;
  long long* dbg;
  EpiArgs epi;
};

enum EpiKind {
  EPI_GATE = 0,
  EPI_RES = 1,
  EPI_BIAS_ACT = 2,
  EPI_CE = 3,
  EPI_MOL = 4,
  EPI_SCALE_RELUMASK = 5,
  EPI_GATE_BWD = 6,
  EPI_DX = 7,
  EPI_LSTM = 8,
  EPI_TOUT = 9,
};


struct WgradTile {
  int a_map, a_ch0, a_shift, a_layer;
  int b_map, b_ch0, b_shift, b_layer;
  long long out_off;
  int ldc;
  int m_valid, n_valid;
  float scale;
  int accumulate;
  const float* div;
};
struct WgradArgs {
  CUtensorMap map[6];
  const WgradTile* tiles;
  float* out;
  int T, B;
};

struct ChainTicket {
  int kind, layer, m, n;
  int dep_lo, dep_hi, dep_target;
  int done;
};

struct ChainArgs {
  const GemmArgs* args;
  const ChainTicket* tix;
  int n_tix, L;
  int* ctr;
  int* err;
  long long* dbg;
  const float* params;
  const unsigned long long* d_step;
  unsigned long long seed;
  int save;
};

}
```

tacotron-2_b200/csrc/t2_tacotron.cu:

```cuda
#include <stdlib.h>
#include <math.h>
#include <stdio.h>
#include <string.h>

#include <string>
#include <vector>

#include "../../include/t2b200.h"
#include "t2_batchnorm.h"
#include "t2_common.cuh"
#include "t2_gemm.h"
#include "t2_params.h"

namespace t2 {
namespace {

typedef __nv_bfloat16 bf16;

struct ConvL {
  int cin, cout, k, act;
  ConvBnParams p;
  long long k_w, k_wT;
  int cinp;
  long long w_y, w_x;
// ... 662 lines not shown
};

int lstm_step(const StepCtx& s, const void* wrec, int H, int K, const void* state, int B, const float* pre, int pre_stride, const float* bias,
              const float* c_prev, float* c_out, const bf16* h_prev, int ld_hp, bf16* h_state, int ld_hs, bf16* h_out, int ld_ho,
              bf16* gst, bf16* tst, const int* lens, int t, int stream_id, float zone, int out_lo = 0, int out_state = 0) {
  ActGemmCall g;
  memset(&g, 0, sizeof(g));
  const int split = s.lo->c.split_bf16;
  if (split) {
    g.a[0] = make_act(wrec, 3 * K, 4 * H, 1, 1, 3 * K); g.na = 1;
    g.seg[0] = Seg{0, 0, 0, 2 * K / kBK, 0, 1}; g.seg[1] = Seg{0, 0, 2 * K, K / kBK, 0, 1}; g.nseg = 2;
    g.w = state; g.wN = B; g.wK = 3 * K; g.wL = 1;
    gst = nullptr; tst = nullptr;
    g.epi.i[2] = out_lo; g.epi.i[10] = K; g.epi.i[11] = out_state ? 2 : 1;
  } else {
  g.a[0] = make_act(wrec, K, 4 * H, 1, 1, K); g.na = 1;
  g.seg[0] = Seg{0, 0, 0, K / kBK, 0, 1}; g.nseg = 1;
  g.w = state; g.wN = B; g.wK = K; g.wL = 1;
  }
  g.T = 4 * H; g.B = 1; g.n_tiles = (B + 31) / 32;
  g.epi.ptr[0] = const_cast<float*>(pre); g.epi.ptr[1] = const_cast<float*>(bias); g.epi.ptr[2] = const_cast<float*>(c_prev); g.epi.ptr[3] = c_out;
  g.epi.ptr[4] = const_cast<bf16*>(h_prev); g.epi.ptr[5] = h_state; g.epi.ptr[6] = h_out; g.epi.ptr[7] = gst; g.epi.ptr[8] = tst;
  g.epi.ptr[9] = const_cast<int*>(lens); g.epi.ptr[10] = const_cast<unsigned long long*>(s.d_step);
  g.epi.i[0] = H; g.epi.i[1] = B; g.epi.i[3] = pre_stride; g.epi.i[4] = ld_hp; g.epi.i[5] = ld_hs; g.epi.i[6] = ld_ho; g.epi.i[7] = t;
  g.epi.i[8] = stream_id; g.epi.i[9] = s.training; g.epi.f[0] = zone; g.epi.seed = s.seed;
  return launch_act_gemm(EPI_LSTM, 32, g, s.st);
}

int conv_block_fwd(const StepCtx& s, const ConvL& L, const void* x_in, long long T, int training) {
  const TL& lo = *s.lo;
  int shifts[8];
  for (int j = 0; j < L.k; ++j) shifts[j] = conv_tap_shift(L.k, j);
  const int split = lo.c.split_bf16;
  bf16* y = reinterpret_cast<bf16*>(s.ws + L.w_y);
  float* yf = reinterpret_cast<float*>(s.ws + L.w_y);
  int rc = conv_gemm(x_in, L.cin, T, lo.B, s.pk + L.k_w, L.cout, L.k * L.cinp * (split ? 3 : 1), L.k, shifts, L.cout % 256 == 0 ? 256 : 128,
                     const_cast<float*>(s.params + L.p.bias), L.act, split ? nullptr : y,
                     split ? yf : nullptr, L.cout, L.cout, 0.f, 0, 0, nullptr, s.st, split);
  if (rc) return rc;
  float* stats = reinterpret_cast<float*>(s.ws + L.w_stats);
  const long long rows = (long long)lo.B * T;
  float* pp = const_cast<float*>(s.params);
  bf16* x = reinterpret_cast<bf16*>(s.ws + L.w_x);
  const BnDropout drop{lo.c.dropout_rate, s.seed, s.d_step, L.stream};
  if (training) T2_CHECK_CUDA(cudaMemsetAsync(stats, 0, 2 * L.cout * sizeof(float), s.st));
  if (split)
    bn_fwd(yf, L.cout, 0, x, 1, nullptr, nullptr, stats, L.cout, s.params + L.p.gamma, s.params + L.p.beta, pp + L.p.mm, pp + L.p.mv, rows, L.cout,
           training, drop, 256, s.st);
  else
    bn_fwd(y, L.cout, 0, x, 0, nullptr, nullptr, stats, L.cout, s.params + L.p.gamma, s.params + L.p.beta, pp + L.p.mm, pp + L.p.mv, rows, L.cout,
           training, drop, 256, s.st);
  T2_CHECK_CUDA(cudaGetLastError());
  return T2_OK;
}


struct WgL { std::vector<WgradTile> tiles; };
enum { WG_PP = 0, WG_POST0 = 1  };
void build_tiles(const TL& lo, std::vector<WgL>& L) {
  L.clear();
  const int H = lo.H, D = lo.D, K1r = 2 * H + D, K2 = 2 * D, PIK = D + 2 * H;
  auto conv = [&](const ConvL& c) { WgL w; append_conv_wgrad_tiles(w.tiles, c.k, 0, c.cin, 0, c.cout, c.p.kernel); L.push_back(w); };
  { WgL w; append_wgrad_tiles(w.tiles, dense_proto(0, 1), 0, lo.PC, 0, lo.M, lo.p_ppk, lo.M); L.push_back(w); }
  for (int i = int(lo.post.size()) - 1; i >= 0; --i) conv(lo.post[i]);
  { WgL w; append_wgrad_tiles(w.tiles, dense_proto(0, 1), 0, PIK, 0, lo.M, lo.p_fk, lo.M); append_wgrad_tiles(w.tiles, dense_proto(0, 1), 0, PIK, lo.M, 1, lo.p_sk, 1); L.push_back(w); }
  { WgL w;
    append_wgrad_tiles(w.tiles, dense_proto(0, 1), 0, K2, 0, 4 * D, lo.p_l2k, 4 * D);
    append_wgrad_tiles(w.tiles, dense_proto(2, 3), 0, K1r, 0, 4 * D, lo.p_l1k + (long long)lo.P2 * 4 * D, 4 * D);
    append_wgrad_tiles(w.tiles, dense_proto(4, 3), 0, lo.P2, 0, 4 * D, lo.p_l1k, 4 * D);
    L.push_back(w); }
  { WgL w;
    append_wgrad_tiles(w.tiles, dense_proto(0, 1), 0, lo.P1, 0, lo.P2, lo.p_p2k, lo.P2);
    append_wgrad_tiles(w.tiles, dense_proto(2, 3), 0, lo.M, 0, lo.P1, lo.p_p1k, lo.P1);
    append_wgrad_tiles(w.tiles, dense_proto(4, 5), 0, D, 0, lo.A, lo.p_qry, lo.A);
    L.push_back(w); }
  { WgL w; append_wgrad_tiles(w.tiles, dense_proto(0, 1), 0, 2 * H, 0, lo.A, lo.p_mem, lo.A); L.push_back(w); }
  for (int d = 0; d < 2; ++d) {
    WgL w;
    append_wgrad_tiles(w.tiles, dense_proto(0, 1), 0, H, 0, 4 * H, lo.p_elk[d] + (long long)lo.C * 4 * H, 4 * H);
    L.push_back(w);
    WgL w2; append_wgrad_tiles(w2.tiles, dense_proto(0, 1), 0, lo.C, 0, 4 * H, lo.p_elk[d], 4 * H); L.push_back(w2);
  }
  for (int i = int(lo.enc.size()) - 1; i >= 0; --i) conv(lo.enc[i]);
}

__global__ void loss_seed_kernel(const float* __restrict__ dec_f, const float* __restrict__ resid, const float* __restrict__ mel,
                                 const float* __restrict__ tgt, bf16* __restrict__ dmel, float* __restrict__ ddec, long long npos, int M,
                                 int clip, float lo, float hi, const int* __restrict__ tlen, int To, const float* __restrict__ scal,
                                 const float* __restrict__ extra) {
  const long long e = blockIdx.x * (long long)blockDim.x + threadIdx.x;
  if (e >= npos * 128) return;
  const long long pos = e / 128; const int m = int(e % 128);
  float g = 0.f;
  if (m < M) {
    const long long o = pos * M + m;
    const float n = scal[5];
    const float raw = dec_f[o] + resid[pos * 128 + m];
    const bool masked = tlen && int(pos % To) >= tlen[pos / To];
    g = masked ? 0.f : 2.f * (mel[o] - tgt[o]) / n;
    if (extra) g += extra[o];
    if (clip && (raw < lo || raw > hi)) g = 0.f;
    ddec[o] = g + (masked ? 0.f : 2.f * (dec_f[o] - tgt[o]) / n);
  }
  dmel[e] = __float2bfloat16(g);
}
__global__ void ddec_tm_kernel(const float* __restrict__ ddec, const bf16* __restrict__ dpost, const float* __restrict__ projo,
                               const float* __restrict__ stop_tgt, bf16* __restrict__ out, int B, int To, int M, int clip, float lo, float hi,
                               const int* __restrict__ tlen, float pos_w, const float* __restrict__ scal, int t0, int t1,
                               const float* __restrict__ fb, const int* __restrict__ choice) {
  const long long e = (long long)t0 * B * 128 + blockIdx.x * (long long)blockDim.x + threadIdx.x;
  if (e >= (long long)t1 * B * 128) return;
  const int m = int(e % 128), b = int((e / 128) % B), t = int(e / (128LL * B));
  float g = 0.f;
  if (m < M) {
    const long long o = ((long long)b * To + t) * M + m;
    g = ddec[o] + __bfloat162float(dpost[o]);
    const float raw = projo[((long long)t * B + b) * 128 + m];
    if (clip && (raw < lo || raw > hi)) g = 0.f;
    if (fb && !choice[t]) g += fb[(long long)b * M + m];
  } else if (m == M) {
    const float x = projo[((long long)t * B + b) * 128 + M];
    const float z = stop_tgt[(long long)b * To + t];
    if (!tlen) g = (1.f / (1.f + __expf(-x)) - z) / scal[6];
    else if (t < tlen[b]) g = ((1.f - z) - (1.f + (pos_w - 1.f) * z) / (1.f + __expf(x))) / scal[6];
  }
  out[e] = __float2bfloat16(g);
}
__global__ void relu_drop_bwd_kernel(const bf16* __restrict__ d, const bf16* __restrict__ y, bf16* __restrict__ dz, long long n, float p) {
  const long long e = blockIdx.x * (long long)blockDim.x + threadIdx.x;
  if (e < n) dz[e] = __float2bfloat16(__bfloat162float(y[e]) > 0.f ? __bfloat162float(d[e]) / (1.f - p) : 0.f);
}

struct CellBwd {
  float* dh_ext; long long ld_ext;
  int zero_ext;
  float* dhs; float* dcs;
  const bf16* gst; const bf16* tst; const float* c_prev;
  bf16* dg_a; long long ld_a;
  bf16* dg_b; long long ld_b;
  const int* lens; int t, B, H, stream;
  float zone; unsigned long long seed; const unsigned long long* step;
};
__global__ void lstm_cell_bwd_kernel(CellBwd a) {
  pdl_wait();
  pdl_launch_dependents();
  const long long e = blockIdx.x * (long long)blockDim.x + threadIdx.x;
  if (e >= (long long)a.B * a.H) return;
  const int b = int(e / a.H), u = int(e % a.H);
  unsigned long long seed = a.seed + (a.step ? *a.step : 0ull);
  const bool live = a.lens ? (a.t < a.lens[b]) : true;
  float dzi = 0.f, dzj = 0.f, dzf = 0.f, dzo = 0.f;
  if (live) {
    const bf16* g = a.gst + (long long)b * 4 * a.H;
    const float gi = __bfloat162float(g[u]), gj = __bfloat162float(g[a.H + u]), gf = __bfloat162float(g[2 * a.H + u]),
                go = __bfloat162float(g[3 * a.H + u]);
    const float tc = __bfloat162float(a.tst[e]);
    const uint64_t idx = (uint64_t(a.t) * a.B + b) * a.H + u;
    const bool mc = a.zone <= 0.f || hash_uniform32(hash_seed(seed, uint32_t(a.stream) * 2u), idx) >= a.zone;
    const bool mh = a.zone <= 0.f || hash_uniform32(hash_seed(seed, uint32_t(a.stream) * 2u + 1u), idx) >= a.zone;
    const float dhs = a.dhs[e], dcs = a.dcs[e];
    const float dh_new = a.dh_ext[(long long)b * a.ld_ext + u] + (mh ? dhs : 0.f);
    if (a.zero_ext) a.dh_ext[(long long)b * a.ld_ext + u] = 0.f;
    const float dc_new = (mc ? dcs : 0.f) + dh_new * go * (1.f - tc * tc);
    dzo = dh_new * tc * go * (1.f - go);
    dzi = dc_new * gj * gi * (1.f - gi);
    dzj = dc_new * gi * (1.f - gj * gj);
// ... 322 lines not shown
                                   float* __restrict__ dvalues, int B, int Ti, int To, int C2) {
  const int b = blockIdx.y, j = blockIdx.x;
  const bool live = j < lens[b];
  for (int c = threadIdx.x; c < C2; c += blockDim.x) {
    float acc = dvalues[((long long)b * Ti + j) * C2 + c];
    if (live) for (int t = 0; t < To; ++t) acc += alpha[((long long)t * B + b) * Ti + j] * __bfloat162float(dctx[((long long)t * B + b) * C2 + c]);
    dvalues[((long long)b * Ti + j) * C2 + c] = live ? acc : 0.f;
  }
}
using AttBwdFn = void (*)(AttBwd);
AttBwdFn att_bwd_fn(int unmasked, int noncumulative) {
  return unmasked ? (noncumulative ? att_bwd_kernel<false, false> : att_bwd_kernel<false, true>)
                  : (noncumulative ? att_bwd_kernel<true, false> : att_bwd_kernel<true, true>);
}
int att_bwd_setup(size_t smem, int unmasked, int noncumulative) {
  T2_CHECK_CUDA(cudaFuncSetAttribute(att_bwd_fn(unmasked, noncumulative), cudaFuncAttributeMaxDynamicSharedMemorySize, int(smem)));
  return T2_OK;
}
int launch_att_bwd(const AttBwd& a, size_t smem, cudaStream_t st) {
  T2_CHECK_CUDA(launch_pdl(att_bwd_fn(a.unmasked, a.noncumulative), dim3(a.B), dim3(kAttThreads), smem, st, a)); t2_count_launch();
  return T2_OK;
}
int launch_cell_bwd(const CellBwd& c, cudaStream_t st) {
  T2_CHECK_CUDA(launch_pdl(lstm_cell_bwd_kernel, dim3(grid1d((long long)c.B * c.H)), dim3(256), 0, st, c)); t2_count_launch();
  return T2_OK;
}
void launch_att_finish(const float* acc, const float* K, const float* bK, const float* Wl, float* grads, int B, int KA, int F, int A, long long o_k,
                       long long o_bk, long long o_wl, long long o_v, long long o_ba, float* scratch, cudaStream_t st) {
  att_finish_kernel<<<grid1d((long long)(KA + 2) * A), 256, 0, st>>>(acc, K, bK, Wl, grads, B, KA, F, A, o_k, o_bk, o_wl, o_v, o_ba, scratch); t2_count_launch();
  att_finish2_kernel<<<grid1d(KA * F + F * A + F + A), 256, 0, st>>>(scratch, K, bK, Wl, grads, KA, F, A, o_k, o_bk, o_wl, o_v, o_ba); t2_count_launch();
}
void launch_dvalues_ctx(const float* alpha, const bf16* dctx, const int* lens, float* dvalues, int B, int Ti, int To, int C2, cudaStream_t st) {
  dvalues_ctx_kernel<<<dim3(Ti, B), 256, 0, st>>>(alpha, dctx, lens, dvalues, B, Ti, To, C2); t2_count_launch();
}

int conv_block_bwd(const StepCtx& s, const ConvL& L, const void* x_in, long long T, const bf16* dout, bf16* dpre, bf16* dx, float* grads,
                   const WgradTile* tiles, int ntiles) {
  const TL& lo = *s.lo;
  const long long rows = (long long)lo.B * T;
  float* stats = reinterpret_cast<float*>(s.ws + L.w_stats);
  const bf16* y = reinterpret_cast<const bf16*>(s.ws + L.w_y);
  float* bsum = stats + 4 * L.cout;
  T2_CHECK_CUDA(cudaMemsetAsync(bsum, 0, 2 * L.cout * sizeof(float), s.st));
  bn_bwd(dout, L.cout, y, L.cout, 0, stats, L.cout, bsum, s.params + L.p.gamma, dpre, L.cout, grads + L.p.gamma, grads + L.p.beta, rows, L.cout, L.act,
         BnDropout{lo.c.dropout_rate, s.seed, s.d_step, L.stream}, 256, s.st);
  colsum(dpre, rows, L.cout, L.cout, grads + L.p.bias, 256, s.st);
  T2_CHECK_CUDA(cudaGetLastError());
  ActT maps[2] = {make_act(x_in, L.cin, int(T), lo.B), make_act(dpre, L.cout, int(T), lo.B)};
  int rc = launch_wgrad(maps, 2, tiles, ntiles, grads, int(T), lo.B, s.st);
  if (rc) return rc;
  if (dx) {
    int shifts[8];
    for (int j = 0; j < L.k; ++j) shifts[j] = -conv_tap_shift(L.k, j);
    rc = conv_gemm(dpre, L.cout, T, lo.B, s.pk + L.k_wT, L.cin, L.k * L.cout, L.k, shifts, L.cin % 256 == 0 ? 256 : 128, nullptr, 0, dx, nullptr, L.cin,
                   L.cin, 0.f, 0, 0, nullptr, s.st);
    if (rc) return rc;
  }
  return T2_OK;
}

}
}

using namespace t2;

extern "C" int t2_taco_sizes(const t2_taco_config_t* cfg, long long* n_params, long long* packed_bytes, long long* workspace_bytes,
                             int* n_tensors) {
  TL lo;
  int rc = build(cfg, lo, nullptr);
  if (rc) return rc;
  if (n_params) *n_params = lo.n_params;
  if (packed_bytes) *packed_bytes = lo.packed_bytes;
  if (workspace_bytes) *workspace_bytes = lo.workspace_bytes;
  if (n_tensors) *n_tensors = int(lo.params.size());
  return T2_OK;
}

extern "C" int t2_taco_param_info(const t2_taco_config_t* cfg, int i, char* name, int cap, long long* offset, int* ndim, int* shape4,
                                  int* trainable) {
  TL lo;
  int rc = build(cfg, lo, nullptr);
  if (rc) return rc;
  return param_info(lo.params, i, name, cap, offset, ndim, shape4, trainable);
}

extern "C" int t2_taco_init(const t2_taco_config_t* cfg, void* d_packed, void* d_workspace, void* stream) {
  TL lo;
  std::vector<PackJob> jobs;
  int rc = build(cfg, lo, &jobs);
  if (rc) return rc;
  cudaStream_t st = static_cast<cudaStream_t>(stream);
  uint8_t* ws = static_cast<uint8_t*>(d_workspace);
  T2_CHECK_CUDA(cudaMemsetAsync(d_packed, 0, lo.packed_bytes, st));
  T2_CHECK_CUDA(cudaMemsetAsync(d_workspace, 0, lo.workspace_bytes, st));
  T2_CHECK_CUDA(cudaMemcpyAsync(ws + lo.w_packjobs, jobs.data(), jobs.size() * sizeof(PackJob), cudaMemcpyHostToDevice, st));
  rc = upload_reg_table(lo.params, ws + lo.w_regtab, st);
  if (rc) return rc;
  std::vector<WgL> wl;
  build_tiles(lo, wl);
  std::vector<WgradTile> all;
  for (auto& w : wl) all.insert(all.end(), w.tiles.begin(), w.tiles.end());
  T2_REQUIRE(all.size() <= 16384, T2_ERR_UNSUPPORTED_SHAPE, "too many weight-gradient tiles (%d)", int(all.size()));
  T2_CHECK_CUDA(cudaMemcpyAsync(ws + lo.w_tiles, all.data(), all.size() * sizeof(WgradTile), cudaMemcpyHostToDevice, st));
  T2_CHECK_CUDA(cudaStreamSynchronize(st));
  return T2_OK;
}

extern "C" int t2_taco_pack_weights(const t2_taco_config_t* cfg, const float* d_params, void* d_packed, void* d_workspace, void* stream) {
  TL lo;
  int rc = build(cfg, lo, nullptr);
  if (rc) return rc;
  return launch_pack(d_params, d_packed, reinterpret_cast<const PackJob*>(static_cast<uint8_t*>(d_workspace) + lo.w_packjobs), lo.n_packjobs,
                     32, 32, static_cast<cudaStream_t>(stream));
}

static int encoder_fwd(const StepCtx& s, const int* d_inputs, const int* d_input_lengths, int training) {
  const TL& lo = *s.lo;
  uint8_t* ws = s.ws; const uint8_t* pk = s.pk; const float* d_params = s.params; cudaStream_t st = s.st;
  const int B = lo.B, Ti = lo.Ti, H = lo.H;
  int rc;
  bf16* emb = reinterpret_cast<bf16*>(ws + lo.w_emb);
  embed_fwd_kernel<<<grid1d((long long)B * Ti * lo.E), 256, 0, st>>>(d_inputs, d_params + lo.p_emb, emb, (long long)B * Ti, lo.E, lo.c.split_bf16); t2_count_launch();
  const void* x = emb;
  for (auto& L : lo.enc) { rc = conv_block_fwd(s, L, x, Ti, training); if (rc) return rc; x = ws + L.w_x; }
  SideStream* side = side_stream();
  if (side) {
    T2_CHECK_CUDA(cudaEventRecord(side->fork, st));
    T2_CHECK_CUDA(cudaStreamWaitEvent(side->s, side->fork, 0));
  }
  for (int d = 0; d < 2; ++d) {
    cudaStream_t sx = (d == 1 && side) ? side->s : st;
    StepCtx sc = s; sc.st = sx;
    float* pre = reinterpret_cast<float*>(ws + lo.w_encpre[d]);
    rc = conv_gemm(x, lo.C, Ti, B, pk + lo.k_encWx[d], 4 * H, lo.C * (lo.c.split_bf16 ? 3 : 1), 1, nullptr, 256, const_cast<float*>(d_params) + lo.p_elb[d], 0,
                   nullptr, pre, 4 * H, 4 * H, 0.f, 0, 0, nullptr, sx, lo.c.split_bf16);
    if (rc) return rc;
    bf16* hh = reinterpret_cast<bf16*>(ws + lo.w_ench[d]);
    float* cc = reinterpret_cast<float*>(ws + lo.w_encc[d]);
    const int hw = lo.c.split_bf16 ? 3 * H : H;
    T2_CHECK_CUDA(cudaMemsetAsync(hh, 0, (size_t)B * hw * 2, sx));
    T2_CHECK_CUDA(cudaMemsetAsync(cc, 0, (size_t)B * H * 4, sx));
    bf16* memory = reinterpret_cast<bf16*>(ws + lo.w_memory);
    for (int sidx = 0; sidx < Ti; ++sidx) {
      const int t = d == 0 ? sidx : Ti - 1 - sidx;
      rc = lstm_step(sc, pk + lo.k_encWr[d], H, H, hh + (long long)sidx * B * hw, B, pre + (long long)t * 4 * H, Ti * 4 * H, nullptr,
                     cc + (long long)sidx * B * H, cc + (long long)(sidx + 1) * B * H, hh + (long long)sidx * B * hw, hw,
                     hh + (long long)(sidx + 1) * B * hw, hw, memory + (long long)t * lo.ld_mem + d * H, Ti * lo.ld_mem,
                     reinterpret_cast<bf16*>(ws + lo.w_encg[d]) + (long long)sidx * B * 4 * H,
                     reinterpret_cast<bf16*>(ws + lo.w_enct[d]) + (long long)sidx * B * H, d_input_lengths, t, 52 + d, lo.c.zoneout_rate,
                     2 * H, 0);
      if (rc) return rc;
    }
  }
  if (side) {
    T2_CHECK_CUDA(cudaEventRecord(side->join, side->s));
    T2_CHECK_CUDA(cudaStreamWaitEvent(st, side->join, 0));
  }
  bf16* values = reinterpret_cast<bf16*>(ws + lo.w_values);
  mask_values_kernel<<<grid1d((long long)B * Ti * lo.ld_mem), 256, 0, st>>>(reinterpret_cast<bf16*>(ws + lo.w_memory), d_input_lengths, values, B, Ti,
                                                                        lo.ld_mem);
  t2_count_launch();
  float* keys = reinterpret_cast<float*>(ws + lo.w_keys);
  return conv_gemm(values, 2 * H, Ti, B, pk + lo.k_mem, lo.A, 2 * H * (lo.c.split_bf16 ? 3 : 1), 1, nullptr, 128, nullptr, 0, nullptr, keys, lo.A, lo.A,
                   0.f, 0, 0, nullptr, st, lo.c.split_bf16);
}

// ... 801 lines not shown
```

tacotron-2_b200/csrc/t2_wavenet.cu:

```cuda
#include <stdlib.h>
#include <math.h>
#include <stdio.h>
#include <string.h>

#include <algorithm>
#include <cmath>
#include <mutex>
#include <string>
#include <vector>

#include "../../include/t2b200.h"
#include "t2_common.cuh"
#include "t2_gemm.h"
#include "t2_params.h"

namespace t2 {
namespace {

typedef __nv_bfloat16 bf16;

struct ColsumJob {
  long long src_off;
  long long rows;
  int C, ld;
  long long dst_off, dst2_off;
  float scale;
  int div_scalar;
};

struct Layout {
  t2_wn_config_t c;
  int L, R, G, Gh, S, C, O, Q, B, T, Tc, Kg, ldo, Op;
  int kw;
  bool split;
  int xm;
  bool scalar_in, mol, gauss;
  int Gi, NS;
  float res_scale;
  std::vector<float> skip_scale;
  std::vector<Param> params;
  long long n_params;
  long long p_in_k, p_in_b, p_f1_k, p_f1_b, p_f2_k, p_f2_b;
  std::vector<long long> p_dil_k, p_dil_b, p_c_k, p_c_b, p_s_k, p_s_b, p_o_k, p_o_b, p_up_k, p_up_b;
  std::vector<long long> p_g_k, p_g_b;
  long long p_emb;
  long long layer_stride;
  long long k_Wg, k_Wo, k_Ws, k_Wf1, k_Wf2, k_WozT, k_WdT, k_WcT, k_Wf1T, k_Wf2T, k_bias_g, k_bias_skip;
  long long packed_bytes;
  long long w_cup, w_x, w_xd, w_ta, w_sb, w_z, w_h1, w_h2, w_dlog, w_dh2, w_dskip, w_dxin, w_dg, w_dcup;
  long long w_skipsum;
  long long w_spk;
  long long w_gbias;
  long long w_gsum;
  long long w_gfx;
  long long w_upgrad[2], w_scalars, w_tiles_main, w_tiles_head, w_packjobs, w_colsum, w_tables;
  std::vector<long long> w_upout;
  std::vector<int> up_w;
  long long workspace_bytes;
  int n_tiles_main, n_tiles_head, n_packjobs, n_colsum;
  std::vector<PackJob> packjobs;
  std::vector<ColsumJob> colsums;
  std::vector<WgradTile> tiles_main, tiles_head;
  std::vector<int> tile_start;
  int MT;
  int n_chain[2];
  long long w_chain_ctr[2], w_chain_tix[2], w_chain_args[2], w_chain_err;
  int dil(int l) const { return 1 << (l % (L / c.stacks)); }
};

void build_chain(const Layout& lo, int dir, std::vector<ChainTicket>& v) {
  const int tpb = (lo.T + kBM - 1) / kBM;
  auto idx = [&](int kind, int l, int m) { return (kind * lo.L + l) * lo.MT + m; };
  const int ng = lo.G / 256;
  const int nz = lo.Gh / (lo.Gh >= 256 ? 256 : 128);
  v.clear();
  v.reserve(lo.n_chain[dir]);
  if (dir == 0) {
    for (int l = 0; l < lo.L; ++l) {
      const int k = ((lo.kw - 1) * lo.dil(l) + kBM - 1) / kBM;
      for (int n = 0; n < ng; ++n)
        for (int m = 0; m < lo.MT; ++m) {
          const int m0 = m / tpb * tpb;
          ChainTicket t{0, l, m, n, 0, -1, 0, idx(0, l, m)};
          if (l > 0) { t.dep_lo = idx(1, l - 1, std::max(m0, m - k)); t.dep_hi = idx(1, l - 1, m); t.dep_target = 1; }
          v.push_back(t);
        }
      if (l + 1 < lo.L)
        for (int m = 0; m < lo.MT; ++m) v.push_back(ChainTicket{1, l, m, 0, idx(0, l, m), idx(0, l, m), ng, idx(1, l, m)});
    }
    return;
  }
  for (int l = lo.L - 1; l >= 0; --l) {
    const int k = ((lo.kw - 1) * lo.dil(l) + kBM - 1) / kBM;
    for (int n = 0; n < nz; ++n)
      for (int m = 0; m < lo.MT; ++m) {
        ChainTicket t{0, l, m, n, 0, -1, 0, idx(0, l, m)};
        if (l + 1 < lo.L) { t.dep_lo = t.dep_hi = idx(1, l + 1, m); t.dep_target = 1; }
        v.push_back(t);
      }
    for (int m = 0; m < lo.MT; ++m) {
      const int m1 = m / tpb * tpb + tpb - 1;
      v.push_back(ChainTicket{1, l, m, 0, idx(0, l, m), idx(0, l, std::min(m1, m + k)), nz, idx(1, l, m)});
    }
  }
}

int build_layout(const t2_wn_config_t* cfg, Layout& lo) {
  T2_REQUIRE(cfg != nullptr, T2_ERR_INVALID_ARG, "null config");
  lo.c = *cfg;
  lo.L = cfg->layers; lo.R = cfg->residual_channels; lo.G = cfg->gate_channels; lo.Gh = lo.G / 2;
  lo.S = cfg->skip_out_channels; lo.C = cfg->cin_channels; lo.O = cfg->out_channels;
  lo.Q = cfg->quantize_channels; lo.B = cfg->B; lo.T = cfg->T; lo.Tc = cfg->Tc;
  lo.split = cfg->split_bf16 != 0;
  lo.xm = lo.split ? 2 : 1;
  T2_REQUIRE(!lo.split || cfg->dropout == 0.f, T2_ERR_INVALID_ARG, "split_bf16 (fp32-class forward) needs dropout = 0");
  lo.scalar_in = cfg->input_type != 2;
  lo.mol = lo.scalar_in;
  T2_REQUIRE(lo.L >= 1 && cfg->stacks >= 1 && lo.L % cfg->stacks == 0, T2_ERR_INVALID_ARG, "layers %% stacks != 0");
  T2_REQUIRE(cfg->kernel_size >= 2 && cfg->kernel_size <= 4, T2_ERR_UNSUPPORTED_SHAPE, "kernel_size must be 2, 3 or 4 (got %d)",
             cfg->kernel_size);
  lo.kw = cfg->kernel_size;
  T2_REQUIRE(lo.R == 128 || lo.R == 256, T2_ERR_UNSUPPORTED_SHAPE, "residual_channels must be 128 or 256 (got %d)", lo.R);
  T2_REQUIRE(lo.S == 128 || lo.S == 256, T2_ERR_UNSUPPORTED_SHAPE, "skip_out_channels must be 128 or 256 (got %d)", lo.S);
  T2_REQUIRE(lo.Gh == 128 || lo.Gh == 256, T2_ERR_UNSUPPORTED_SHAPE, "gate_channels must be 256 or 512 (got %d)", lo.G);
  T2_REQUIRE(lo.C == 0 || (lo.C % 8 == 0 && lo.C <= 128), T2_ERR_UNSUPPORTED_SHAPE, "cin_channels must be 0 or a multiple of 8 <= 128");
  lo.gauss = lo.scalar_in && lo.O == 2;
  if (lo.mol) {
    T2_REQUIRE(lo.gauss || (lo.O % 3 == 0 && lo.O >= 3 && lo.O <= 30), T2_ERR_UNSUPPORTED_SHAPE,
               "scalar input needs out_channels = 2 (Gaussian) or 3 * nr_mix <= 30 (mixture of logistics), got %d", lo.O);
  } else {
    T2_REQUIRE(lo.O == 256 && lo.Q == 256, T2_ERR_UNSUPPORTED_SHAPE, "mulaw-quantize needs out_channels == quantize_channels == 256");
  }
  T2_REQUIRE(lo.B >= 1 && lo.T >= 1, T2_ERR_INVALID_ARG, "bad B/T");
  lo.Gi = cfg->gin_channels; lo.NS = cfg->n_speakers;
  T2_REQUIRE(lo.Gi >= 0 && (lo.Gi == 0 || lo.NS >= 1), T2_ERR_INVALID_ARG,
             "gin_channels must be >= 0, and n_speakers >= 1 when gin_channels > 0 (got %d / %d)", lo.Gi, lo.NS);
  T2_REQUIRE(cfg->upsample_type >= 0 && cfg->upsample_type <= 2, T2_ERR_INVALID_ARG,
             "upsample_type must be 0 (SubPixel), 1 (2D) or 2 (1D), got %d", cfg->upsample_type);
  T2_REQUIRE(cfg->upsample_activation >= 0 && cfg->upsample_activation <= 2, T2_ERR_INVALID_ARG,
             "upsample_activation must be 0 (ReLU), 1 (LeakyReLU) or 2 (none), got %d", cfg->upsample_activation);
  T2_REQUIRE(cfg->leaky_alpha >= 0.f && cfg->leaky_alpha <= 1.f, T2_ERR_INVALID_ARG, "leaky_alpha must be in [0, 1], got %g",
             double(cfg->leaky_alpha));
// ... 69 lines not shown
  lo.k_Wg = pk.take(L * lo.G * lo.Kg * km * 2);
  lo.k_Wo = pk.take(L * lo.R * lo.Gh * km * 2);
  lo.k_Ws = pk.take((long long)lo.S * L * lo.Gh * km * 2);
  lo.k_Wf1 = pk.take((long long)lo.S * lo.S * km * 2);
  lo.k_Wf2 = pk.take((long long)(lo.O < 32 ? 32 : lo.O) * lo.S * km * 2);
  lo.k_WozT = pk.take(L * lo.Gh * (lo.R + lo.S) * 2);
  lo.k_WdT = pk.take(L * lo.R * lo.kw * lo.G * 2);
  lo.k_WcT = pk.take((long long)(lo.C > 0 ? lo.C : 8) * L * lo.G * 2);
  lo.k_Wf1T = pk.take((long long)lo.S * lo.S * 2);
  lo.k_Wf2T = pk.take((long long)lo.S * lo.Op * 2);
  lo.k_bias_g = pk.take(L * lo.G * 4);
  lo.k_bias_skip = pk.take(lo.S * 4);
  lo.packed_bytes = pk.used;
  Arena ws;
  const long long BT = (long long)lo.B * lo.T;
  lo.w_cup = ws.take(BT * (lo.split ? 256 : (lo.C > 0 ? lo.C : 8)) * 2);
  lo.w_upout.clear();
  for (size_t i = 0; i < lo.up_w.size(); ++i) lo.w_upout.push_back(ws.take((long long)lo.B * lo.C * lo.up_w[i] * 4));
  lo.w_upgrad[0] = ws.take(BT * (lo.C > 0 ? lo.C : 8) * 4);
  lo.w_upgrad[1] = ws.take(BT * (lo.C > 0 ? lo.C : 8) * 4);
  lo.w_x = ws.take(L * BT * lo.R * 2 * lo.xm);
  lo.w_xd = cfg->dropout > 0.f ? ws.take(L * BT * lo.R * 2) : lo.w_x;
  lo.w_ta = ws.take(L * BT * lo.Gh * 2);
  lo.w_sb = ws.take(L * BT * lo.Gh * 2);
  lo.w_z = ws.take(L * BT * lo.Gh * 2 * lo.xm);
  lo.w_h1 = ws.take(BT * lo.S * 2 * lo.xm);
  lo.w_h2 = ws.take(BT * lo.S * 2 * lo.xm);
  lo.w_dlog = ws.take(BT * lo.ldo * 2);
  lo.w_dh2 = ws.take(BT * lo.S * 2);
  lo.w_dskip = ws.take(BT * lo.S * 2);
  lo.w_dxin = ws.take(L * BT * lo.R * 2);
  lo.w_dg = ws.take(L * BT * lo.G * 2);
  lo.w_dcup = ws.take(BT * (lo.C > 0 ? lo.C : 8) * 4);
  lo.w_scalars = ws.take(64 * 4);
  lo.w_skipsum = ws.take(lo.S * 8);
  lo.w_gfx = ws.take(lo.n_params * 8);

  lo.packjobs.clear();
  std::vector<PackJob>& pj = lo.packjobs;
  for (int l = 0; l < lo.L; ++l) {
    const long long wg = lo.k_Wg + (long long)l * lo.G * lo.Kg * km * 2;
    if (lo.split) {
      const int R = lo.R, Gh = lo.Gh;
      for (int j = 0; j < lo.kw; ++j)
        add_pack_split(pj, lo.p_dil_k[l] + (long long)j * R * lo.G, R, lo.G, wg, 3 * lo.Kg, j * 3 * R, j * 3 * R + 2 * R, R, 1.f, Gh);
      const int kc = 3 * lo.kw * R;
      if (lo.C > 0) add_pack_split(pj, lo.p_c_k[l], lo.C, lo.G, wg, 3 * lo.Kg, kc, kc + 256, 128, 1.f, Gh);
      add_pack_split(pj, lo.p_o_k[l], Gh, R, lo.k_Wo + (long long)l * R * Gh * 3 * 2, 3 * Gh, 0, 2 * Gh, Gh);
      add_pack_split(pj, lo.p_s_k[l], Gh, lo.S, lo.k_Ws, 3 * lo.L * Gh, l * 2 * Gh, 2 * lo.L * Gh + l * Gh, Gh, lo.skip_scale[l]);
    } else {
    for (int j = 0; j < lo.kw; ++j) add_pack(pj, lo.p_dil_k[l] + (long long)j * lo.R * lo.G, lo.R, lo.G, wg, lo.Kg, 1, j * lo.R, 1.f, lo.Gh);
    if (lo.C > 0) add_pack(pj, lo.p_c_k[l], lo.C, lo.G, wg, lo.Kg, 1, lo.kw * lo.R, 1.f, lo.Gh);
    add_pack(pj, lo.p_o_k[l], lo.Gh, lo.R, lo.k_Wo + (long long)l * lo.R * lo.Gh * 2, lo.Gh, 1, 0);
    add_pack(pj, lo.p_s_k[l], lo.Gh, lo.S, lo.k_Ws, lo.L * lo.Gh, 1, l * lo.Gh, lo.skip_scale[l]);
    }
    const long long woz = lo.k_WozT + (long long)l * lo.Gh * (lo.R + lo.S) * 2;
    add_pack(pj, lo.p_o_k[l], lo.Gh, lo.R, woz, lo.R + lo.S, 0, 0, lo.res_scale);
    add_pack(pj, lo.p_s_k[l], lo.Gh, lo.S, woz, lo.R + lo.S, 0, lo.R, lo.skip_scale[l]);
    const long long wd = lo.k_WdT + (long long)l * lo.R * lo.kw * lo.G * 2;
    for (int j = 0; j < lo.kw; ++j) add_pack(pj, lo.p_dil_k[l] + (long long)j * lo.R * lo.G, lo.R, lo.G, wd, lo.kw * lo.G, 0, j * lo.G);
    if (lo.C > 0) add_pack(pj, lo.p_c_k[l], lo.C, lo.G, lo.k_WcT, lo.L * lo.G, 0, l * lo.G);
  }
  if (lo.split) {
    add_pack_split(pj, lo.p_f1_k, lo.S, lo.S, lo.k_Wf1, 3 * lo.S, 0, 2 * lo.S, lo.S);
    add_pack_split(pj, lo.p_f2_k, lo.S, lo.O, lo.k_Wf2, 3 * lo.S, 0, 2 * lo.S, lo.S);
  } else {
    add_pack(pj, lo.p_f1_k, lo.S, lo.S, lo.k_Wf1, lo.S, 1, 0);
    add_pack(pj, lo.p_f2_k, lo.S, lo.O, lo.k_Wf2, lo.S, 1, 0);
  }
  add_pack(pj, lo.p_f1_k, lo.S, lo.S, lo.k_Wf1T, lo.S, 0, 0);
  add_pack(pj, lo.p_f2_k, lo.S, lo.O, lo.k_Wf2T, lo.Op, 0, 0);
  if (!lo.mol) add_pack(pj, lo.p_f2_k, lo.S, lo.O, lo.k_Wf2T, lo.Op, 0, 256);
  lo.n_packjobs = int(lo.packjobs.size());

  lo.tiles_main.clear();
  auto proto = [](int am, int ash, int al, int bm, int bl, float scale) {
    WgradTile t; memset(&t, 0, sizeof(t));
    t.a_map = am; t.a_shift = ash; t.a_layer = al; t.b_map = bm; t.b_layer = bl; t.scale = scale;
    return t;
  };
  lo.tile_start.assign(lo.L + 1, 0);
  for (int l = 0; l < lo.L; ++l) {
    const int d = lo.dil(l);
    lo.tile_start[l] = int(lo.tiles_main.size());
    for (int j = 0; j < lo.kw; ++j)
      append_wgrad_tiles(lo.tiles_main, proto(0, -(lo.kw - 1 - j) * d, l, 1, l, 1.f), 0, lo.R, 0, lo.G, lo.p_dil_k[l] + (long long)j * lo.R * lo.G, lo.G);
    if (lo.C > 0) append_wgrad_tiles(lo.tiles_main, proto(2, 0, 0, 1, l, 1.f), 0, lo.C, 0, lo.G, lo.p_c_k[l], lo.G);
    for (int m0 = 0; m0 < lo.Gh; m0 += 128) {
      if (l < lo.L - 1)
        append_wgrad_tiles(lo.tiles_main, proto(3, 0, l, 4, l + 1, lo.res_scale), m0, 128, 0, lo.R, lo.p_o_k[l] + (long long)m0 * lo.R, lo.R);
      append_wgrad_tiles(lo.tiles_main, proto(3, 0, l, 5, 0, lo.skip_scale[l]), m0, 128, 0, lo.S, lo.p_s_k[l] + (long long)m0 * lo.S, lo.S);
    }
  }
  lo.tiles_head.clear();
  WgradTile f2 = proto(2, 0, 0, 3, 0, 1.f);
  f2.accumulate = 2;
  f2.div = reinterpret_cast<const float*>(1);
  for (int m0 = 0; m0 < lo.S; m0 += 128) {
    append_wgrad_tiles(lo.tiles_head, proto(0, 0, 0, 1, 0, 1.f), m0, 128, 0, lo.S, lo.p_f1_k + (long long)m0 * lo.S, lo.S);
    for (int part = 0; part < (lo.mol ? 1 : 2); ++part)
      append_wgrad_tiles(lo.tiles_head, f2, m0, 128, part * 256, lo.O, lo.p_f2_k + (long long)m0 * lo.O, lo.O);
  }
  lo.n_tiles_main = int(lo.tiles_main.size());
  lo.tile_start[lo.L] = lo.n_tiles_main;
  lo.n_tiles_head = int(lo.tiles_head.size());

  lo.colsums.clear();
  auto cs = [&](long long src, long long rows, int C, int ld, long long dst, long long dst2, float scale, int div) {
    ColsumJob j; j.src_off = src; j.rows = rows; j.C = C; j.ld = ld; j.dst_off = dst; j.dst2_off = dst2; j.scale = scale;
    j.div_scalar = div; lo.colsums.push_back(j);
  };
  cs(lo.w_dlog, BT, lo.O, lo.ldo, lo.p_f2_b, -1, 1.f, 1);
  if (!lo.mol) cs(lo.w_dlog + 256 * 2, BT, lo.O, lo.ldo, lo.p_f2_b, -1, 1.f, 1);
  lo.n_colsum = int(lo.colsums.size());

  lo.w_tiles_main = ws.take((long long)lo.n_tiles_main * sizeof(WgradTile));
  lo.w_tiles_head = ws.take((long long)lo.n_tiles_head * sizeof(WgradTile));
  lo.w_packjobs = ws.take((long long)lo.n_packjobs * sizeof(PackJob));
  lo.w_colsum = ws.take((long long)lo.n_colsum * sizeof(ColsumJob));
  lo.w_tables = ws.take((long long)lo.L * (3 * sizeof(long long) + sizeof(float)));
  lo.MT = lo.B * ((lo.T + kBM - 1) / kBM);
  lo.n_chain[0] = lo.L * (lo.G / 256) * lo.MT + (lo.L - 1) * lo.MT;
  lo.n_chain[1] = lo.L * (lo.Gh / (lo.Gh >= 256 ? 256 : 128)) * lo.MT + lo.L * lo.MT;
  for (int dir = 0; dir < 2; ++dir) {
    lo.w_chain_ctr[dir] = ws.take((16 + 2LL * lo.L * lo.MT) * 4);
    lo.w_chain_tix[dir] = ws.take((long long)lo.n_chain[dir] * sizeof(ChainTicket));
    lo.w_chain_args[dir] = ws.take(2LL * lo.L * sizeof(GemmArgs));
  }
  lo.w_chain_err = ws.take(4);
  lo.w_spk = lo.w_gbias = lo.w_gsum = -1;
  if (lo.Gi > 0) {
    lo.w_spk = ws.take((1LL + lo.B) * 4);
    lo.w_gbias = ws.take(L * lo.B * lo.G * 4);
    lo.w_gsum = ws.take(L * lo.B * lo.G * 8);
  }
  lo.workspace_bytes = ws.used;
  return T2_OK;
}

struct DerivedArgs {
  const float* params;
  float* bias_g;
  float* bias_skip;
  const long long* offs;
  const float* scales;
  int L, G, S;
};
__global__ void derived_bias_kernel(DerivedArgs a) {
  const int i = blockIdx.x * blockDim.x + threadIdx.x;
  if (i < a.L * a.G) {
    const int l = i / a.G, g = i % a.G;
    float v = a.params[a.offs[3 * l] + g];
    if (a.offs[3 * l + 1] >= 0) v += a.params[a.offs[3 * l + 1] + g];
    a.bias_g[i] = v;
  }
  if (i < a.S) {
    float v = 0.f;
    for (int l = 0; l < a.L; ++l) v += a.scales[l] * a.params[a.offs[3 * l + 2] + i];
    a.bias_skip[i] = v;
  }
}

struct GinArgs {
  const float* params;
  const float* bias;
  long long bias_ld;
  const int* on;
  const int* ids;
  float* out;
  long long out_l, out_b;
  long long p_k, p_b, p_stride, p_emb;
  int L, B, G, Gi, NS;
};
__global__ void gin_bias_kernel(GinArgs a) {
  const long long i = blockIdx.x * (long long)blockDim.x + threadIdx.x;
  if (i >= (long long)a.L * a.B * a.G) return;
  const int g = int(i % a.G), b = int((i / a.G) % a.B), l = int(i / ((long long)a.G * a.B));
  float v = a.bias[l * a.bias_ld + g];
  if (a.ids && (!a.on || *a.on)) {
    const int id = a.ids[b];
    float s = __int_as_float(0x7fffffff);
    if (id >= 0 && id < a.NS) {
      const float* W = a.params + a.p_k + l * a.p_stride + g;
      const float* e = a.params + a.p_emb + (long long)id * a.Gi;
      s = a.params[a.p_b + l * a.p_stride + g];
// ... 819 lines not shown
    up1d_bwd_input_kernel<<<dim3((W + kUp1Tw - 1) / kUp1Tw, B), dim3(kUp1Tw, kUp1Rows), smem, st>>>(out, dout, K, din, C, W, s, act, alpha);
  } else {
    upsample_bwd_input_kernel<<<grid1d(4LL * B * C * W), 256, 0, st>>>(out, dout, 0, K, din, B, C, W, s, type, act, alpha);
  }
  t2_count_launch();
  T2_CHECK_CUDA(cudaGetLastError());
  return T2_OK;
}

GinArgs gin_args(const Layout& lo, const float* params) {
  GinArgs a;
  memset(&a, 0, sizeof(a));
  a.params = params;
  a.p_k = lo.p_g_k[0]; a.p_b = lo.p_g_b[0]; a.p_stride = lo.layer_stride; a.p_emb = lo.p_emb;
  a.L = lo.L; a.B = lo.B; a.G = lo.G; a.Gi = lo.Gi; a.NS = lo.NS;
  return a;
}

void launch_derived_bias(const DerivedArgs& a, cudaStream_t st) {
  derived_bias_kernel<<<grid1d(std::max((long long)a.L * a.G, (long long)a.S)), 256, 0, st>>>(a); t2_count_launch();
}
void launch_gin_bias(const GinArgs& a, cudaStream_t st) {
  gin_bias_kernel<<<grid1d((long long)a.L * a.B * a.G), 256, 0, st>>>(a); t2_count_launch();
}
void launch_set_speakers(int* spk, const int* ids, int B, cudaStream_t st) {
  set_speakers_kernel<<<grid1d(B), 256, 0, st>>>(spk, ids, B); t2_count_launch();
}
void launch_gin_wgrad(const GinGradArgs& a, cudaStream_t st) {
  gin_wgrad_kernel<<<grid1d((long long)a.L * a.G), 256, 0, st>>>(a); t2_count_launch();
}
void launch_gin_demb(const GinGradArgs& a, cudaStream_t st) {
  gin_demb_kernel<<<dim3(a.NS, a.Gi), kGinThreads, 0, st>>>(a); t2_count_launch();
}
void launch_first_conv(const void* xin, int scalar_in, const float* W, const float* bias, bf16* x, bf16* xd, long long npos, int R,
                       float p, unsigned long long seed, const unsigned long long* step, int split, cudaStream_t st) {
  first_conv_kernel<<<grid1d(npos * (R / 8)), 256, 0, st>>>(xin, scalar_in, W, bias, x, xd, npos, R, p, seed, step, split); t2_count_launch();
}
void launch_first_conv_bwd(const void* xin, int scalar_in, const bf16* dx0, long long* dW, long long npos, int R, cudaStream_t st) {
  first_conv_bwd_kernel<<<dim3((unsigned)((npos + 63) / 64)), R, 0, st>>>(xin, scalar_in, dx0, dW, npos, R); t2_count_launch();
}
void launch_colsum(const uint8_t* ws, long long* acc, const ColsumJob* jobs, int njobs, const float* scalars, cudaStream_t st) {
  colsum_kernel<<<dim3(96, njobs), 256, 0, st>>>(ws, acc, jobs, scalars); t2_count_launch();
}
void launch_skip_bias(const long long* skipsum, float* grads, const long long* offs, const float* scales, int L, int S, cudaStream_t st) {
  skip_bias_kernel<<<grid1d((long long)L * S), 256, 0, st>>>(skipsum, grads, offs, scales, L, S); t2_count_launch();
}
void launch_cl_to_chw(const float* in, float* out, int B, int T, int C, cudaStream_t st) {
  cl_to_chw_kernel<<<dim3((T + 31) / 32, (C + 31) / 32, B), dim3(32, 8), 0, st>>>(in, out, T, C); t2_count_launch();
}

}

int launch_fx_finalize(const long long* acc, float* out, long long n, cudaStream_t st) {
  if (n <= 0) return T2_OK;
  fx_finalize_kernel<<<unsigned((n + 255) / 256), 256, 0, st>>>(acc, out, n);
  t2_count_launch();
  T2_CHECK_CUDA(cudaGetLastError());
  return T2_OK;
}
}

using namespace t2;

extern "C" int t2_wn_sizes(const t2_wn_config_t* cfg, t2_wn_sizes_t* out) {
  Layout lo;
  int rc = build_layout(cfg, lo);
  if (rc) return rc;
  T2_REQUIRE(out != nullptr, T2_ERR_INVALID_ARG, "null out");
  out->n_params = lo.n_params;
  out->packed_bytes = lo.packed_bytes;
  out->workspace_bytes = lo.workspace_bytes;
  out->n_tensors = int(lo.params.size());
  return T2_OK;
}

extern "C" int t2_wn_param_info(const t2_wn_config_t* cfg, int i, char* name, int name_cap, long long* offset,
                                int* ndim, int* shape4) {
  Layout lo;
  int rc = build_layout(cfg, lo);
  if (rc) return rc;
  return param_info(lo.params, i, name, name_cap, offset, ndim, shape4, nullptr);
}

extern "C" int t2_wn_init(const t2_wn_config_t* cfg, void* d_packed, void* d_workspace, void* stream) {
  Layout lo;
  int rc = build_layout(cfg, lo);
  if (rc) return rc;
  cudaStream_t st = static_cast<cudaStream_t>(stream);
  uint8_t* ws = static_cast<uint8_t*>(d_workspace);
  T2_CHECK_CUDA(cudaMemsetAsync(d_packed, 0, lo.packed_bytes, st));
  T2_CHECK_CUDA(cudaMemsetAsync(d_workspace, 0, lo.workspace_bytes, st));
  chain_cache_forget(d_workspace, lo.workspace_bytes);
  float* scalars = reinterpret_cast<float*>(ws + lo.w_scalars);
  for (auto& t : lo.tiles_head)
    if (t.div != nullptr) t.div = scalars + 1;
  T2_CHECK_CUDA(cudaMemcpyAsync(ws + lo.w_tiles_main, lo.tiles_main.data(), lo.tiles_main.size() * sizeof(WgradTile), cudaMemcpyHostToDevice, st));
  T2_CHECK_CUDA(cudaMemcpyAsync(ws + lo.w_tiles_head, lo.tiles_head.data(), lo.tiles_head.size() * sizeof(WgradTile), cudaMemcpyHostToDevice, st));
  T2_CHECK_CUDA(cudaMemcpyAsync(ws + lo.w_packjobs, lo.packjobs.data(), lo.packjobs.size() * sizeof(PackJob), cudaMemcpyHostToDevice, st));
  T2_CHECK_CUDA(cudaMemcpyAsync(ws + lo.w_colsum, lo.colsums.data(), lo.colsums.size() * sizeof(ColsumJob), cudaMemcpyHostToDevice, st));
  std::vector<long long> offs(3 * lo.L);
  for (int l = 0; l < lo.L; ++l) {
    offs[3 * l] = lo.p_dil_b[l];
    offs[3 * l + 1] = lo.C > 0 ? lo.p_c_b[l] : -1;
    offs[3 * l + 2] = lo.p_s_b[l];
  }
  T2_CHECK_CUDA(cudaMemcpyAsync(ws + lo.w_tables, offs.data(), offs.size() * sizeof(long long), cudaMemcpyHostToDevice, st));
  T2_CHECK_CUDA(cudaMemcpyAsync(ws + lo.w_tables + 3 * lo.L * sizeof(long long), lo.skip_scale.data(), lo.L * sizeof(float),
                                cudaMemcpyHostToDevice, st));
  T2_CHECK_CUDA(cudaStreamSynchronize(st));
  return T2_OK;
}

extern "C" int t2_wn_pack_weights(const t2_wn_config_t* cfg, const float* d_params, void* d_packed,
                                  void* d_workspace, void* stream) {
  Layout lo;
  int rc = build_layout(cfg, lo);
  if (rc) return rc;
  cudaStream_t st = static_cast<cudaStream_t>(stream);
  uint8_t* ws = static_cast<uint8_t*>(d_workspace);
  uint8_t* pk = static_cast<uint8_t*>(d_packed);
  rc = launch_pack(d_params, pk, reinterpret_cast<const PackJob*>(ws + lo.w_packjobs), lo.n_packjobs, 128, 16, st);
  if (rc) return rc;
  long long* d_offs = reinterpret_cast<long long*>(ws + lo.w_tables);
  float* d_scales = reinterpret_cast<float*>(ws + lo.w_tables + 3 * lo.L * sizeof(long long));
  DerivedArgs a;
  a.params = d_params; a.bias_g = reinterpret_cast<float*>(pk + lo.k_bias_g); a.bias_skip = reinterpret_cast<float*>(pk + lo.k_bias_skip);
  a.offs = d_offs; a.scales = d_scales; a.L = lo.L; a.G = lo.G; a.S = lo.S;
  launch_derived_bias(a, st);
  T2_CHECK_CUDA(cudaGetLastError());
  return T2_OK;
}

extern "C" int t2_wn_forward(const t2_wn_config_t* cfg, const float* d_params, const void* d_packed,
                             void* d_workspace, const void* d_x, const float* d_c, const void* d_targets,
                             const int* d_lengths, float* d_loss, float* d_logits, int save_for_backward,
                             unsigned long long seed, const unsigned long long* d_step, void* stream) {
  Layout lo;
  int rc = build_layout(cfg, lo);
  if (rc) return rc;
  cudaStream_t st = static_cast<cudaStream_t>(stream);
  uint8_t* ws = static_cast<uint8_t*>(d_workspace);
  const uint8_t* pk = static_cast<const uint8_t*>(d_packed);
  const long long BT = (long long)lo.B * lo.T;
  float* scalars = reinterpret_cast<float*>(ws + lo.w_scalars);
  const float p = cfg->dropout;
  T2_CHECK_CUDA(cudaMemsetAsync(scalars, 0, 16 * sizeof(float), st));

  T2_REQUIRE(!lo.split || (!save_for_backward && !cfg->c_pre_upsampled), T2_ERR_INVALID_ARG,
             "split_bf16 (fp32-class) mode is forward / loss only (save_for_backward = 0) and needs the upsampling net");
  if (lo.Gi > 0) {
    GinArgs a = gin_args(lo, d_params);
    const int* spk = reinterpret_cast<const int*>(ws + lo.w_spk);
    a.bias = reinterpret_cast<const float*>(pk + lo.k_bias_g); a.bias_ld = lo.G;
    a.on = spk; a.ids = spk + 1;
    a.out = reinterpret_cast<float*>(ws + lo.w_gbias); a.out_l = (long long)lo.B * lo.G; a.out_b = lo.G;
    launch_gin_bias(a, st);
    T2_CHECK_CUDA(cudaGetLastError());
  }
  bf16* c_up = reinterpret_cast<bf16*>(ws + lo.w_cup);
  if (lo.split) T2_CHECK_CUDA(cudaMemsetAsync(c_up, 0, (size_t)BT * 256 * 2, st));
  if (lo.C > 0) {
    T2_REQUIRE(d_c != nullptr, T2_ERR_INVALID_ARG, "local conditioning enabled but d_c is NULL");
    if (cfg->c_pre_upsampled) {
      launch_f32_to_bf16(d_c, c_up, BT * lo.C, st);
    } else {
      const float* in = d_c;
// ... 113 lines not shown
    uint8_t* ws = static_cast<uint8_t*>(d_workspace);
    const int g = phase - 1;
    const int l0 = int((long long)lo.L * g / n_groups), l1 = int((long long)lo.L * (g + 1) / n_groups);
    const int t0 = lo.tile_start[l0], t1 = lo.tile_start[l1];
    ActT maps[6] = {make_act(ws + lo.w_xd, lo.R, lo.T, lo.B, lo.L), make_act(ws + lo.w_dg, lo.G, lo.T, lo.B, lo.L),
                    make_act(ws + lo.w_cup, lo.C > 0 ? lo.C : 8, lo.T, lo.B, 1),
                    make_act(ws + lo.w_z, lo.Gh, lo.T, lo.B, lo.L), make_act(ws + lo.w_dxin, lo.R, lo.T, lo.B, lo.L),
                    make_act(ws + lo.w_dskip, lo.S, lo.T, lo.B, 1)};
    return launch_wgrad(maps, 6, reinterpret_cast<const WgradTile*>(ws + lo.w_tiles_main) + t0, t1 - t0, d_grads, lo.T, lo.B, st);
  }
  if (phase == 100) {
    SideStream* side = side_stream();
    if (side) {
      T2_CHECK_CUDA(cudaEventRecord(side->join, side->s));
      T2_CHECK_CUDA(cudaStreamWaitEvent(st, side->join, 0));
    }
    return launch_fx_finalize(reinterpret_cast<const long long*>(static_cast<uint8_t*>(d_workspace) + lo.w_gfx), d_grads, lo.n_params, st);
  }
  uint8_t* ws = static_cast<uint8_t*>(d_workspace);
  const uint8_t* pk = static_cast<const uint8_t*>(d_packed);
  const long long BT = (long long)lo.B * lo.T;
  float* scalars = reinterpret_cast<float*>(ws + lo.w_scalars);
  const float p = cfg->dropout;
  T2_CHECK_CUDA(cudaMemsetAsync(d_grads, 0, lo.n_params * sizeof(float), st));
  T2_CHECK_CUDA(cudaMemsetAsync(ws + lo.w_skipsum, 0, lo.S * sizeof(long long), st));
  T2_CHECK_CUDA(cudaMemsetAsync(ws + lo.w_gfx, 0, lo.n_params * sizeof(long long), st));
  if (lo.Gi > 0) T2_CHECK_CUDA(cudaMemsetAsync(ws + lo.w_gsum, 0, (size_t)lo.L * lo.B * lo.G * sizeof(long long), st));
  long long* gfx = reinterpret_cast<long long*>(ws + lo.w_gfx);
  bf16* h1 = reinterpret_cast<bf16*>(ws + lo.w_h1);
  bf16* h2 = reinterpret_cast<bf16*>(ws + lo.w_h2);
  bf16* dlog = reinterpret_cast<bf16*>(ws + lo.w_dlog);
  bf16* dh2 = reinterpret_cast<bf16*>(ws + lo.w_dh2);
  bf16* dskip = reinterpret_cast<bf16*>(ws + lo.w_dskip);
  bf16* dxin = reinterpret_cast<bf16*>(ws + lo.w_dxin);
  bf16* dg = reinterpret_cast<bf16*>(ws + lo.w_dg);
  bf16* ta_all = reinterpret_cast<bf16*>(ws + lo.w_ta);
  bf16* sb_all = reinterpret_cast<bf16*>(ws + lo.w_sb);
  {
    ActGemmCall g;
    memset(&g, 0, sizeof(g));
    g.a[0] = make_act(dlog, lo.ldo, lo.T, lo.B); g.na = 1;
    g.seg[0] = Seg{0, 0, 0, lo.Op / kBK, 0, 1}; g.nseg = 1;
    g.w = pk + lo.k_Wf2T; g.wN = lo.S; g.wK = lo.Op; g.wL = 1;
    g.T = lo.T; g.B = lo.B; g.n_tiles = 1;
    g.epi.ptr[0] = dh2; g.epi.ptr[1] = h2; g.epi.ptr[2] = scalars + 1; g.epi.f[0] = 1.f; g.epi.i[0] = lo.S;
    g.epi.ptr[3] = gfx + lo.p_f1_b;
    rc = launch_act_gemm(EPI_SCALE_RELUMASK, lo.S, g, st);
    if (rc) return rc;
  }
  {
    ActGemmCall g;
    memset(&g, 0, sizeof(g));
    g.a[0] = make_act(dh2, lo.S, lo.T, lo.B); g.na = 1;
    g.seg[0] = Seg{0, 0, 0, lo.S / kBK, 0, 1}; g.nseg = 1;
    g.w = pk + lo.k_Wf1T; g.wN = lo.S; g.wK = lo.S; g.wL = 1;
    g.T = lo.T; g.B = lo.B; g.n_tiles = 1;
    g.epi.ptr[0] = dskip; g.epi.ptr[1] = h1; g.epi.ptr[2] = nullptr; g.epi.f[0] = 1.f; g.epi.i[0] = lo.S;
    g.epi.ptr[3] = ws + lo.w_skipsum;
    rc = launch_act_gemm(EPI_SCALE_RELUMASK, lo.S, g, st);
    if (rc) return rc;
  }
  launch_skip_bias(reinterpret_cast<const long long*>(ws + lo.w_skipsum), d_grads, reinterpret_cast<const long long*>(ws + lo.w_tables),
                   reinterpret_cast<const float*>(ws + lo.w_tables + 3 * lo.L * sizeof(long long)), lo.L, lo.S, st);
  SideStream* side = side_stream();
  cudaStream_t sb = st;
  if (side) {
    T2_CHECK_CUDA(cudaEventRecord(side->fork, st));
    T2_CHECK_CUDA(cudaStreamWaitEvent(side->s, side->fork, 0));
    sb = side->s;
  }
  {
    ActT hmaps[4] = {make_act(h1, lo.S, lo.T, lo.B), make_act(dh2, lo.S, lo.T, lo.B), make_act(h2, lo.S, lo.T, lo.B),
                     make_act(dlog, lo.ldo, lo.T, lo.B)};
    rc = launch_wgrad(hmaps, 4, reinterpret_cast<const WgradTile*>(ws + lo.w_tiles_head), lo.n_tiles_head, d_grads, lo.T, lo.B, sb);
    if (rc) return rc;
    launch_colsum(ws, gfx, reinterpret_cast<const ColsumJob*>(ws + lo.w_colsum), lo.n_colsum, scalars, sb);
    T2_CHECK_CUDA(cudaGetLastError());
  }
  const ActT a_dxin = make_act(dxin, lo.R, lo.T, lo.B, lo.L);
  const ActT a_dskip = make_act(dskip, lo.S, lo.T, lo.B, 1);
  const ActT a_dg = make_act(dg, lo.G, lo.T, lo.B, lo.L);
  const int bn_z = lo.Gh >= 256 ? 256 : 128;
  if (use_chain(lo)) {
    rc = launch_chain(lo, 1, ws, pk, d_params, 1, seed, d_step, side ? lo.n_tiles_head : 0, st);
    if (rc) return rc;
  } else {
    for (int l = lo.L - 1; l >= 0; --l) {
      ActGemmCall gz = make_dz_call(lo, ws, pk, l, gfx);
      rc = launch_act_gemm(EPI_GATE_BWD, bn_z, gz, st);
      if (rc) return rc;
      ActGemmCall gx = make_dx_call(lo, ws, pk, l, p, seed, d_step, gfx);
      rc = launch_act_gemm(EPI_DX, lo.R, gx, st);
      if (rc) return rc;
    }
  }
  if (lo.Gi > 0) {
    GinGradArgs a;
    a.params = d_params; a.spk = reinterpret_cast<const int*>(ws + lo.w_spk);
    a.S = reinterpret_cast<const long long*>(ws + lo.w_gsum); a.gfx = gfx; a.grads = d_grads;
    a.offs = reinterpret_cast<const long long*>(ws + lo.w_tables);
    a.p_k = lo.p_g_k[0]; a.p_b = lo.p_g_b[0]; a.p_stride = lo.layer_stride; a.p_emb = lo.p_emb;
    a.L = lo.L; a.B = lo.B; a.G = lo.G; a.Gi = lo.Gi; a.NS = lo.NS;
    launch_gin_wgrad(a, st);
    launch_gin_demb(a, st);
    T2_CHECK_CUDA(cudaGetLastError());
  }
  if (side) {
    T2_CHECK_CUDA(cudaEventRecord(side->fork2, st));
    T2_CHECK_CUDA(cudaStreamWaitEvent(side->s, side->fork2, 0));
  }
  if (phase == -1) {
    ActT maps[6] = {make_act(ws + lo.w_xd, lo.R, lo.T, lo.B, lo.L), a_dg,
                    make_act(ws + lo.w_cup, lo.C > 0 ? lo.C : 8, lo.T, lo.B, 1),
                    make_act(ws + lo.w_z, lo.Gh, lo.T, lo.B, lo.L), a_dxin, a_dskip};
    rc = launch_wgrad(maps, 6, reinterpret_cast<const WgradTile*>(ws + lo.w_tiles_main), lo.n_tiles_main, d_grads, lo.T, lo.B, st);
    if (rc) return rc;
  }
  launch_first_conv_bwd(d_x, lo.scalar_in ? 1 : 0, dxin, gfx + lo.p_in_k, BT, lo.R, sb);
  T2_CHECK_CUDA(cudaGetLastError());
  if (lo.C > 0 && !cfg->c_pre_upsampled) {
    float* dcup = reinterpret_cast<float*>(ws + lo.w_dcup);
    ActGemmCall g;
    memset(&g, 0, sizeof(g));
    g.a[0] = a_dg; g.na = 1;
    g.seg[0] = Seg{0, 0, 0, lo.G / kBK, 0, lo.L}; g.nseg = 1;
    g.w = pk + lo.k_WcT; g.wN = lo.C; g.wK = lo.L * lo.G; g.wL = 1;
    g.T = lo.T; g.B = lo.B; g.n_tiles = 1;
    g.epi.ptr[0] = nullptr; g.epi.ptr[1] = nullptr; g.epi.ptr[2] = dcup;
    g.epi.i[0] = lo.C; g.epi.i[1] = 0; g.epi.i[2] = lo.C;
    rc = launch_act_gemm(EPI_BIAS_ACT, 128, g, sb);
    if (rc) return rc;
    float* dchw = reinterpret_cast<float*>(ws + lo.w_upgrad[1]);
    launch_cl_to_chw(dcup, dchw, lo.B, lo.T, lo.C, sb);
    const float* dout = dchw;
    int pp = 0;
    for (int i = int(lo.up_w.size()) - 1; i >= 0; --i) {
      const int s = cfg->upsample_scales[i];
      const int W = lo.up_w[i] / s;
      const float* layer_in = i == 0 ? d_c : reinterpret_cast<const float*>(ws + lo.w_upout[i - 1]);
      const float* out = reinterpret_cast<const float*>(ws + lo.w_upout[i]);
      rc = launch_upsample_bwd_param(layer_in, out, dout, gfx + lo.p_up_k[i], gfx + lo.p_up_b[i], lo.B, lo.C, W, s, cfg->upsample_type,
                                     cfg->upsample_activation, cfg->leaky_alpha, sb);
      if (rc) return rc;
      if (i > 0) {
        float* din = reinterpret_cast<float*>(ws + lo.w_upgrad[pp]);
        rc = launch_upsample_bwd_input(out, dout, d_params + lo.p_up_k[i], din, lo.B, lo.C, W, s, cfg->upsample_type, cfg->upsample_activation,
                                       cfg->leaky_alpha, sb);
        if (rc) return rc;
        dout = din;
        pp ^= 1;
      }
    }
  }
  if (side && phase == -1) {
    T2_CHECK_CUDA(cudaEventRecord(side->join, sb));
    T2_CHECK_CUDA(cudaStreamWaitEvent(st, side->join, 0));
  }
  if (phase == -1) {
    const int rc = launch_fx_finalize(gfx, d_grads, lo.n_params, st);
    if (rc) return rc;
  }
  return T2_OK;
}

extern "C" int t2_dbg_wn_per_layer(int mode) {
  T2_REQUIRE(mode >= 0 && mode <= 2, T2_ERR_INVALID_ARG, "dbg_wn_per_layer: mode must be 0, 1 or 2 (got %d)", mode);
  g_chain_mode = mode;
// ... 998 lines not shown
```

Measured before the change: 3.743 million.

## Pair wgrad tiles into 2-CTA clusters sharing operand loads via TMA multicast

Weight-gradient tiles that share the same A or B operand are paired into 2-CTA clusters. Each CTA issues half of the shared operand loads with TMA multicast, and the empty barriers are signalled remotely in both CTAs. This cuts redundant global and L2 reads of activation maps in the wgrad GEMMs. In exchange it adds cluster scheduling constraints, cluster syncs, and padding slots where a tile has no partner.

Result: no change. 3.757 million, median of 6 (+0.4%).

```diff
diff --git a/include/t2b200.h b/include/t2b200.h
--- a/include/t2b200.h
+++ b/include/t2b200.h
@@ -61,6 +61,7 @@
 } t2_dbg_wgrad_tile_t;
 int t2_dbg_wgrad_tiles(const t2_dbg_act_t* maps, int nmaps, const t2_dbg_wgrad_tile_t* tiles, int ntiles, float* d_out, int T, int B,
                        void* stream);
+int t2_wgrad_max_active_pairs(void);
 int t2_dbg_fx_colsum(const float* d_addends, int nrows, int ncols, float* d_out, void* stream);
 
 typedef struct {
@@ -128,6 +129,7 @@
 int t2_wn_sizes(const t2_wn_config_t* cfg, t2_wn_sizes_t* out);
 int t2_wn_param_info(const t2_wn_config_t* cfg, int i, char* name, int name_cap, long long* offset, int* ndim,
                      int* shape4);
+int t2_wn_wgrad_stats(const t2_wn_config_t* cfg, int which, long long* stats);
 int t2_wn_init(const t2_wn_config_t* cfg, void* d_packed, void* d_workspace, void* stream);
 int t2_wn_pack_weights(const t2_wn_config_t* cfg, const float* d_params, void* d_packed, void* d_workspace,
                        void* stream);
@@ -198,6 +200,7 @@
 
 int t2_taco_sizes(const t2_taco_config_t* cfg, long long* n_params, long long* packed_bytes, long long* workspace_bytes,
                   int* n_tensors);
+int t2_taco_wgrad_stats(const t2_taco_config_t* cfg, long long* stats);
 int t2_taco_param_info(const t2_taco_config_t* cfg, int i, char* name, int name_cap, long long* offset, int* ndim,
                        int* shape4, int* trainable);
 int t2_taco_init(const t2_taco_config_t* cfg, void* d_packed, void* d_workspace, void* stream);
@@ -246,6 +249,7 @@
   int split_bf16;
 } t2_cbhg_config_t;
 int t2_cbhg_sizes(const t2_cbhg_config_t* cfg, long long* n_params, long long* packed_bytes, long long* workspace_bytes, int* n_tensors);
+int t2_cbhg_wgrad_stats(const t2_cbhg_config_t* cfg, long long* stats);
 int t2_cbhg_param_info(const t2_cbhg_config_t* cfg, int i, char* name, int name_cap, long long* offset, int* ndim, int* shape4,
                        int* trainable);
 int t2_cbhg_init(const t2_cbhg_config_t* cfg, void* d_packed, void* d_workspace, void* stream);
diff --git a/tacotron-2_b200/csrc/t2_api.cu b/tacotron-2_b200/csrc/t2_api.cu
--- a/tacotron-2_b200/csrc/t2_api.cu
+++ b/tacotron-2_b200/csrc/t2_api.cu
@@ -55,6 +55,7 @@
   proto.a_map = 0; proto.a_shift = shift_a; proto.b_map = 1; proto.scale = scale;
   std::vector<WgradTile> tiles;
   append_wgrad_tiles(tiles, proto, 0, Ca, 0, Cb, 0, Cb);
+  tiles = pair_wgrad_tiles(tiles.data(), int(tiles.size()));
   WgradTile* dt = nullptr;
   cudaStream_t st = static_cast<cudaStream_t>(stream);
   T2_CHECK_CUDA(cudaMallocAsync(&dt, tiles.size() * sizeof(WgradTile), st));
@@ -111,16 +112,19 @@
                tiles[i].m_valid >= 1 && tiles[i].m_valid <= 128 && tiles[i].n_valid >= 1 && tiles[i].n_valid <= 256 &&
                tiles[i].accumulate >= 0 && tiles[i].accumulate <= 2,
                T2_ERR_INVALID_ARG, "wgrad_tiles: bad tile %d", i);
+  const std::vector<WgradTile> slots = pair_wgrad_tiles(reinterpret_cast<const WgradTile*>(tiles), ntiles);
   WgradTile* dt = nullptr;
   cudaStream_t st = static_cast<cudaStream_t>(stream);
-  T2_CHECK_CUDA(cudaMallocAsync(&dt, ntiles * sizeof(WgradTile), st));
-  const cudaError_t e = cudaMemcpyAsync(dt, tiles, ntiles * sizeof(WgradTile), cudaMemcpyHostToDevice, st);
-  int rc = e == cudaSuccess ? launch_wgrad(reinterpret_cast<const ActT*>(maps), nmaps, dt, ntiles, d_out, T, B, st)
+  T2_CHECK_CUDA(cudaMallocAsync(&dt, slots.size() * sizeof(WgradTile), st));
+  const cudaError_t e = cudaMemcpyAsync(dt, slots.data(), slots.size() * sizeof(WgradTile), cudaMemcpyHostToDevice, st);
+  int rc = e == cudaSuccess ? launch_wgrad(reinterpret_cast<const ActT*>(maps), nmaps, dt, int(slots.size()), d_out, T, B, st)
                             : t2_set_error(T2_ERR_CUDA, "wgrad_tiles: tile table upload failed: %s", cudaGetErrorString(e));
   cudaStreamSynchronize(st);
   cudaFreeAsync(dt, st);
   return rc;
 }
+
+extern "C" int t2_wgrad_max_active_pairs(void) { return t2::wgrad_max_active_pairs(); }
 
 __global__ void fx_colsum_kernel(const float* __restrict__ v, long long n, int ncols, long long* acc) {
   const long long i = blockIdx.x * (long long)blockDim.x + threadIdx.x;
diff --git a/tacotron-2_b200/csrc/t2_cbhg.cu b/tacotron-2_b200/csrc/t2_cbhg.cu
--- a/tacotron-2_b200/csrc/t2_cbhg.cu
+++ b/tacotron-2_b200/csrc/t2_cbhg.cu
@@ -599,6 +599,7 @@
   { std::vector<WgradTile> w;
     for (int k = 1; k <= lo.K; ++k) append_conv_wgrad_tiles(w, k, 0, lo.M, (k - 1) * lo.CC, lo.CC, lo.bank[k - 1].p.kernel);
     L.push_back(w); }
+  for (auto& w : L) w = pair_wgrad_tiles(w.data(), int(w.size()));
 }
 
 size_t gru_fwd_smem(int split) { return (64 * 256 + 64 * 128) * 4 * (split ? 2 : 1) + 3 * kGruItems * kRU * 4; }
@@ -671,6 +672,22 @@
   int rc = build(cfg, lo, nullptr);
   if (rc) return rc;
   return param_info(lo.params, i, name, cap, offset, ndim, shape4, trainable);
+}
+
+extern "C" int t2_cbhg_wgrad_stats(const t2_cbhg_config_t* cfg, long long* stats) {
+  CL lo;
+  int rc = build(cfg, lo, nullptr);
+  if (rc) return rc;
+  T2_REQUIRE(stats != nullptr, T2_ERR_INVALID_ARG, "wgrad_stats: null stats");
+  std::vector<std::vector<WgradTile>> wl;
+  build_tiles(lo, wl);
+  for (int i = 0; i < 7; ++i) stats[i] = 0;
+  for (const auto& w : wl) {
+    long long st[7];
+    wgrad_slot_stats(w.data(), int(w.size()), st);
+    for (int i = 0; i < 7; ++i) stats[i] += st[i];
+  }
+  return T2_OK;
 }
 
 extern "C" int t2_cbhg_init(const t2_cbhg_config_t* cfg, void* d_packed, void* d_workspace, void* stream) {
diff --git a/tacotron-2_b200/csrc/t2_common.cuh b/tacotron-2_b200/csrc/t2_common.cuh
--- a/tacotron-2_b200/csrc/t2_common.cuh
+++ b/tacotron-2_b200/csrc/t2_common.cuh
@@ -209,6 +209,14 @@
       "l"(reinterpret_cast<uint64_t>(m)), "r"(smem_u32(bar)), "r"(c0), "r"(c1), "r"(c2), "h"(cta_mask)
       : "memory");
 }
+__device__ __forceinline__ void tma_load_4d_mc(void* smem, const CUtensorMap* m, uint64_t* bar, int c0, int c1, int c2, int c3,
+                                               uint16_t cta_mask) {
+  asm volatile(
+      "cp.async.bulk.tensor.4d.shared::cluster.global.tile.mbarrier::complete_tx::bytes.multicast::cluster "
+      "[%0], [%1, {%3, %4, %5, %6}], [%2], %7;\n" ::"r"(smem_u32(smem)),
+      "l"(reinterpret_cast<uint64_t>(m)), "r"(smem_u32(bar)), "r"(c0), "r"(c1), "r"(c2), "r"(c3), "h"(cta_mask)
+      : "memory");
+}
 __device__ __forceinline__ void tma_store_3d(const CUtensorMap* m, const void* smem, int c0, int c1, int c2) {
   asm volatile("cp.async.bulk.tensor.3d.global.shared::cta.bulk_group [%0, {%2, %3, %4}], [%1];\n" ::"l"(reinterpret_cast<uint64_t>(m)),
                "r"(smem_u32(smem)), "r"(c0), "r"(c1), "r"(c2)
@@ -240,6 +248,10 @@
 }
 __device__ __forceinline__ void mbar_arrive_cluster(uint64_t* bar, uint32_t rank) {
   asm volatile("mbarrier.arrive.release.cluster.shared::cluster.b64 _, [%0];\n" ::"r"(mapa_cluster(bar, rank)) : "memory");
+}
+
+__device__ __forceinline__ void mbar_arrive_remote(uint64_t* bar, uint32_t rank) {
+  asm volatile("mbarrier.arrive.shared::cluster.b64 _, [%0];\n" ::"r"(mapa_cluster(bar, rank)) : "memory");
 }
 
 __device__ __forceinline__ void bulk_load_1d(void* smem_dst, const void* gmem_src, uint32_t bytes, uint64_t* bar) {
diff --git a/tacotron-2_b200/csrc/t2_gemm.cu b/tacotron-2_b200/csrc/t2_gemm.cu
--- a/tacotron-2_b200/csrc/t2_gemm.cu
+++ b/tacotron-2_b200/csrc/t2_gemm.cu
@@ -241,16 +241,36 @@
   return t2_set_error(T2_ERR_UNSUPPORTED_SHAPE, "act_gemm: no kernel for epilogue %d with BN=%d", epi, BN);
 }
 
-int launch_wgrad(const ActT* maps, int nmaps, const WgradTile* tiles_dev, int ntiles, float* out, int T,
+static bool wgrad_pairs_enabled() {
+  const char* e = getenv("T2_WGRAD_PAIRS");
+  return !(e && e[0] == '0');
+}
+
+int wgrad_max_active_pairs() {
+  cudaLaunchConfig_t cfg;
+  memset(&cfg, 0, sizeof(cfg));
+  cfg.gridDim = dim3(2); cfg.blockDim = dim3(kGemmThreads); cfg.dynamicSmemBytes = kWgSmemBytes;
+  cudaLaunchAttribute attr;
+  attr.id = cudaLaunchAttributeClusterDimension;
+  attr.val.clusterDim.x = 2; attr.val.clusterDim.y = 1; attr.val.clusterDim.z = 1;
+  cfg.attrs = &attr; cfg.numAttrs = 1;
+  int n = 0;
+  T2_CHECK_CUDA(cudaFuncSetAttribute(wgrad_gemm_kernel, cudaFuncAttributeMaxDynamicSharedMemorySize, kWgSmemBytes));
+  T2_CHECK_CUDA(cudaOccupancyMaxActiveClusters(&n, wgrad_gemm_kernel, &cfg));
+  return n;
+}
+
+int launch_wgrad(const ActT* maps, int nmaps, const WgradTile* slots_dev, int nslots, float* out, int T,
                  int B, cudaStream_t stream) {
-  T2_REQUIRE(nmaps >= 1 && nmaps <= 6 && ntiles >= 1, T2_ERR_INVALID_ARG, "wgrad: bad map/tile count");
+  T2_REQUIRE(nmaps >= 1 && nmaps <= 6 && nslots >= 2 && nslots % 2 == 0, T2_ERR_INVALID_ARG,
+             "wgrad: bad map count %d or slot count %d (slot tables hold pairs)", nmaps, nslots);
   WgradArgs g;
   memset(&g, 0, sizeof(g));
   for (int i = 0; i < 6; ++i) {
     int rc = encode_act_map(&g.map[i], maps[i < nmaps ? i : 0], kBK);
     if (rc) return rc;
   }
-  g.tiles = tiles_dev;
+  g.tiles = slots_dev;
   g.out = out;
   g.T = T;
   g.B = B;
@@ -261,14 +281,75 @@
   }
   cudaLaunchConfig_t cfg;
   memset(&cfg, 0, sizeof(cfg));
-  cfg.gridDim = dim3(ntiles); cfg.blockDim = dim3(kGemmThreads); cfg.dynamicSmemBytes = kWgSmemBytes; cfg.stream = stream;
-  cudaLaunchAttribute attr[1];
-  attr[0].id = cudaLaunchAttributeProgrammaticStreamSerialization;
-  attr[0].val.programmaticStreamSerializationAllowed = 1;
-  cfg.attrs = attr; cfg.numAttrs = pdl_enabled() ? 1 : 0;
+  cfg.gridDim = dim3(nslots); cfg.blockDim = dim3(kGemmThreads); cfg.dynamicSmemBytes = kWgSmemBytes; cfg.stream = stream;
+  cudaLaunchAttribute attr[2];
+  int na = 0;
+  if (pdl_enabled()) {
+    attr[na].id = cudaLaunchAttributeProgrammaticStreamSerialization;
+    attr[na].val.programmaticStreamSerializationAllowed = 1;
+    ++na;
+  }
+  const bool pairs = wgrad_pairs_enabled();
+  if (pairs) {
+    attr[na].id = cudaLaunchAttributeClusterDimension;
+    attr[na].val.clusterDim.x = 2; attr[na].val.clusterDim.y = 1; attr[na].val.clusterDim.z = 1;
+    ++na;
+  }
+  cfg.attrs = attr; cfg.numAttrs = na;
+  if (pairs) {
+    static const int max_pairs = wgrad_max_active_pairs();
+    T2_REQUIRE(max_pairs > 0, T2_ERR_UNSUPPORTED_SHAPE, "wgrad: clusters of 2 CTAs cannot be scheduled on this device");
+  }
   T2_CHECK_CUDA(cudaLaunchKernelEx(&cfg, wgrad_gemm_kernel, g));
   t2_count_launch();
   return T2_OK;
+}
+
+static bool wgrad_same_a(const WgradTile& x, const WgradTile& y) {
+  return x.a_map == y.a_map && x.a_ch0 == y.a_ch0 && x.a_shift == y.a_shift && x.a_layer == y.a_layer;
+}
+static bool wgrad_same_b(const WgradTile& x, const WgradTile& y) {
+  return x.b_map == y.b_map && x.b_ch0 == y.b_ch0 && x.b_shift == y.b_shift && x.b_layer == y.b_layer;
+}
+static int wgrad_nblk(const WgradTile& t) { return (t.n_valid + 63) >> 6; }
+
+std::vector<WgradTile> pair_wgrad_tiles(const WgradTile* tiles, int n) {
+  std::vector<WgradTile> slots;
+  std::vector<char> used(n, 0);
+  for (int i = 0; i < n; ++i) {
+    if (used[i]) continue;
+    used[i] = 1;
+    int j = -1, share = kWgShareNone;
+    for (int k = i + 1; k < n && j < 0; ++k)
+      if (!used[k] && wgrad_nblk(tiles[k]) == wgrad_nblk(tiles[i]) && wgrad_same_b(tiles[i], tiles[k])) { j = k; share = kWgShareB; }
+    for (int k = i + 1; k < n && j < 0; ++k)
+      if (!used[k] && wgrad_nblk(tiles[k]) == wgrad_nblk(tiles[i]) && wgrad_same_a(tiles[i], tiles[k])) { j = k; share = kWgShareA; }
+    WgradTile a = tiles[i], b;
+    memset(&b, 0, sizeof(b));
+    if (j >= 0) { used[j] = 1; b = tiles[j]; }
+    a.share = share; b.share = share;
+    slots.push_back(a);
+    slots.push_back(b);
+  }
+  return slots;
+}
+
+void wgrad_slot_stats(const WgradTile* slots, int nslots, long long* st) {
+  constexpr long long kBlk = kBK * 128;
+  for (int i = 0; i < 7; ++i) st[i] = 0;
+  st[1] = nslots;
+  for (int i = 0; i < nslots; ++i) {
+    const WgradTile& t = slots[i];
+    if (t.m_valid == 0) continue;
+    const long long nb = wgrad_nblk(t);
+    ++st[0];
+    st[4] += 2LL * kWgBM * (64 * nb) * kBK;
+    st[6] += (2 + nb) * kBlk;
+    const bool second = (i & 1) && t.share != kWgShareNone;
+    st[5] += second ? (t.share == kWgShareA ? nb * kBlk : 2 * kBlk) : (2 + nb) * kBlk;
+    if (!(i & 1) && t.share == kWgShareA) ++st[2];
+    if (!(i & 1) && t.share == kWgShareB) ++st[3];
+  }
 }
 
 void append_wgrad_tiles(std::vector<WgradTile>& v, const WgradTile& proto, int a_ch0, int Ca, int b_ch0, int Cb, long long out_off,
diff --git a/tacotron-2_b200/csrc/t2_gemm.cuh b/tacotron-2_b200/csrc/t2_gemm.cuh
--- a/tacotron-2_b200/csrc/t2_gemm.cuh
+++ b/tacotron-2_b200/csrc/t2_gemm.cuh
@@ -1079,7 +1079,7 @@
 
 template <int N>
 __device__ __forceinline__ void wgrad_consume(const WgradArgs& g, const WgradTile& tile, uint8_t* smem, uint64_t* full_bar,
-                                              uint64_t* empty_bar, int total_kb) {
+                                              uint64_t* empty_bar, int total_kb, bool paired) {
   constexpr int kBlk = kBK * 128;
   const int warp = threadIdx.x >> 5, lane = threadIdx.x & 31, wg = warp >> 2;
   float d[N / 2];
@@ -1102,7 +1102,10 @@
     wgmma_commit();
     wgmma_fence_regs(d);
     wgmma_wait<1>();
-    if (kb > 0 && lane == 0) mbar_arrive(&empty_bar[prev]);
+    if (kb > 0 && lane == 0) {
+      if (paired) { mbar_arrive_remote(&empty_bar[prev], 0); mbar_arrive_remote(&empty_bar[prev], 1); }
+      else mbar_arrive(&empty_bar[prev]);
+    }
     prev = stage;
     if (++stage == kWgStages) { stage = 0; phase ^= 1; }
   }
@@ -1136,15 +1139,19 @@
   uint64_t* empty_bar = full_bar + kWgStages;
   const int warp = threadIdx.x >> 5;
   const WgradTile tile = g.tiles[blockIdx.x];
+  if (tile.m_valid == 0) return;
+  const int share = cluster_nctarank() > 1 ? tile.share : int(kWgShareNone);
+  const int crank = int(cluster_ctarank());
   const int kb_per_b = (g.T + kBK - 1) / kBK;
   const int total_kb = kb_per_b * g.B;
   const int nblk = (tile.n_valid + 63) >> 6;
 
   if (warp == 8 && elect_one()) {
-    for (int i = 0; i < kWgStages; ++i) { mbar_init(&full_bar[i], 1); mbar_init(&empty_bar[i], 8); }
+    for (int i = 0; i < kWgStages; ++i) { mbar_init(&full_bar[i], 1); mbar_init(&empty_bar[i], share ? 16 : 8); }
     fence_barrier_init();
   }
   __syncthreads();
+  if (share) cluster_sync_all();
   pdl_wait();
   pdl_launch_dependents();
   constexpr int kBlk = kBK * 128;
@@ -1152,6 +1159,10 @@
   if (warp == 8) {
     if (elect_one()) {
       int stage = 0; uint32_t phase = 0;
+      auto load = [&](uint8_t* dst, int map, int ch, int pos, int bb, int layer, bool shared, int i) {
+        if (!shared) tma_load_4d(dst, &g.map[map], &full_bar[stage], ch, pos, bb, layer);
+        else if ((i & 1) == crank) tma_load_4d_mc(dst, &g.map[map], &full_bar[stage], ch, pos, bb, layer, uint16_t(3));
+      };
       for (int bb = 0; bb < g.B; ++bb)
         for (int kb = 0; kb < kb_per_b; ++kb) {
           mbar_wait(&empty_bar[stage], phase ^ 1);
@@ -1159,21 +1170,26 @@
           uint8_t* sa = smem + stage * kWgStageBytes;
           uint8_t* sb = sa + 2 * kBlk;
           const int tpos = kb * kBK;
-          tma_load_4d(sa, &g.map[tile.a_map], &full_bar[stage], tile.a_ch0, tpos + tile.a_shift, bb, tile.a_layer);
-          tma_load_4d(sa + kBlk, &g.map[tile.a_map], &full_bar[stage], tile.a_ch0 + 64, tpos + tile.a_shift, bb, tile.a_layer);
+          for (int i = 0; i < 2; ++i)
+            load(sa + i * kBlk, tile.a_map, tile.a_ch0 + 64 * i, tpos + tile.a_shift, bb, tile.a_layer, share == kWgShareA, i);
           for (int i = 0; i < nblk; ++i)
-            tma_load_4d(sb + i * kBlk, &g.map[tile.b_map], &full_bar[stage], tile.b_ch0 + 64 * i, tpos + tile.b_shift, bb, tile.b_layer);
+            load(sb + i * kBlk, tile.b_map, tile.b_ch0 + 64 * i, tpos + tile.b_shift, bb, tile.b_layer, share == kWgShareB, i);
           if (++stage == kWgStages) { stage = 0; phase ^= 1; }
         }
     }
   } else {
+    const bool paired = share != kWgShareNone;
     switch (nblk) {
-      case 1: wgrad_consume<64>(g, tile, smem, full_bar, empty_bar, total_kb); break;
-      case 2: wgrad_consume<128>(g, tile, smem, full_bar, empty_bar, total_kb); break;
-      case 3: wgrad_consume<192>(g, tile, smem, full_bar, empty_bar, total_kb); break;
-      default: wgrad_consume<256>(g, tile, smem, full_bar, empty_bar, total_kb); break;
-    }
-  }
-}
-
-}
+      case 1: wgrad_consume<64>(g, tile, smem, full_bar, empty_bar, total_kb, paired); break;
+      case 2: wgrad_consume<128>(g, tile, smem, full_bar, empty_bar, total_kb, paired); break;
+      case 3: wgrad_consume<192>(g, tile, smem, full_bar, empty_bar, total_kb, paired); break;
+      default: wgrad_consume<256>(g, tile, smem, full_bar, empty_bar, total_kb, paired); break;
+    }
+  }
+  if (share) {
+    __syncthreads();
+    cluster_sync_all();
+  }
+}
+
+}
diff --git a/tacotron-2_b200/csrc/t2_gemm.h b/tacotron-2_b200/csrc/t2_gemm.h
--- a/tacotron-2_b200/csrc/t2_gemm.h
+++ b/tacotron-2_b200/csrc/t2_gemm.h
@@ -51,8 +51,11 @@
 int make_gemm_args(int epi, int BN, const ActGemmCall& c, GemmArgs& g, dim3& grid, int& cs);
 int launch_wn_chain(bool fwd, int bn0, int bn1, const ChainArgs& a, int grid, cudaStream_t st);
 long long* take_timing_slice(long long n_slots);
-int launch_wgrad(const ActT* maps, int nmaps, const WgradTile* tiles_dev, int ntiles, float* out,
+int launch_wgrad(const ActT* maps, int nmaps, const WgradTile* slots_dev, int nslots, float* out,
                  int T, int B, cudaStream_t stream);
+int wgrad_max_active_pairs();
+std::vector<WgradTile> pair_wgrad_tiles(const WgradTile* tiles, int n);
+void wgrad_slot_stats(const WgradTile* slots, int nslots, long long* st);
 void append_wgrad_tiles(std::vector<WgradTile>& v, const WgradTile& proto, int a_ch0, int Ca, int b_ch0, int Cb, long long out_off,
                         int ldc);
 WgradTile dense_proto(int am, int bm, int a_shift = 0);
diff --git a/tacotron-2_b200/csrc/t2_gemm_types.h b/tacotron-2_b200/csrc/t2_gemm_types.h
--- a/tacotron-2_b200/csrc/t2_gemm_types.h
+++ b/tacotron-2_b200/csrc/t2_gemm_types.h
@@ -62,8 +62,10 @@
   int m_valid, n_valid;
   float scale;
   int accumulate;
+  int share;
   const float* div;
 };
+enum WgradShare { kWgShareNone = 0, kWgShareA = 1, kWgShareB = 2 };
 struct WgradArgs {
   CUtensorMap map[6];
   const WgradTile* tiles;
diff --git a/tacotron-2_b200/csrc/t2_tacotron.cu b/tacotron-2_b200/csrc/t2_tacotron.cu
--- a/tacotron-2_b200/csrc/t2_tacotron.cu
+++ b/tacotron-2_b200/csrc/t2_tacotron.cu
@@ -768,6 +768,7 @@
     WgL w2; append_wgrad_tiles(w2.tiles, dense_proto(0, 1), 0, lo.C, 0, 4 * H, lo.p_elk[d], 4 * H); L.push_back(w2);
   }
   for (int i = int(lo.enc.size()) - 1; i >= 0; --i) conv(lo.enc[i]);
+  for (WgL& w : L) w.tiles = pair_wgrad_tiles(w.tiles.data(), int(w.tiles.size()));
 }
 
 __global__ void loss_seed_kernel(const float* __restrict__ dec_f, const float* __restrict__ resid, const float* __restrict__ mel,
@@ -1256,6 +1257,22 @@
   int rc = build(cfg, lo, nullptr);
   if (rc) return rc;
   return param_info(lo.params, i, name, cap, offset, ndim, shape4, trainable);
+}
+
+extern "C" int t2_taco_wgrad_stats(const t2_taco_config_t* cfg, long long* stats) {
+  TL lo;
+  int rc = build(cfg, lo, nullptr);
+  if (rc) return rc;
+  T2_REQUIRE(stats != nullptr, T2_ERR_INVALID_ARG, "wgrad_stats: null stats");
+  std::vector<WgL> wl;
+  build_tiles(lo, wl);
+  for (int i = 0; i < 7; ++i) stats[i] = 0;
+  for (const auto& w : wl) {
+    long long st[7];
+    wgrad_slot_stats(w.tiles.data(), int(w.tiles.size()), st);
+    for (int i = 0; i < 7; ++i) stats[i] += st[i];
+  }
+  return T2_OK;
 }
 
 extern "C" int t2_taco_init(const t2_taco_config_t* cfg, void* d_packed, void* d_workspace, void* stream) {
diff --git a/tacotron-2_b200/csrc/t2_wavenet.cu b/tacotron-2_b200/csrc/t2_wavenet.cu
--- a/tacotron-2_b200/csrc/t2_wavenet.cu
+++ b/tacotron-2_b200/csrc/t2_wavenet.cu
@@ -58,6 +58,7 @@
   std::vector<int> up_w;
   long long workspace_bytes;
   int n_tiles_main, n_tiles_head, n_packjobs, n_colsum;
+  int n_head_busy;
   std::vector<PackJob> packjobs;
   std::vector<ColsumJob> colsums;
   std::vector<WgradTile> tiles_main, tiles_head;
@@ -293,15 +294,18 @@
   lo.tile_start.assign(lo.L + 1, 0);
   for (int l = 0; l < lo.L; ++l) {
     const int d = lo.dil(l);
-    lo.tile_start[l] = int(lo.tiles_main.size());
+    std::vector<WgradTile> lt;
     for (int j = 0; j < lo.kw; ++j)
-      append_wgrad_tiles(lo.tiles_main, proto(0, -(lo.kw - 1 - j) * d, l, 1, l, 1.f), 0, lo.R, 0, lo.G, lo.p_dil_k[l] + (long long)j * lo.R * lo.G, lo.G);
-    if (lo.C > 0) append_wgrad_tiles(lo.tiles_main, proto(2, 0, 0, 1, l, 1.f), 0, lo.C, 0, lo.G, lo.p_c_k[l], lo.G);
+      append_wgrad_tiles(lt, proto(0, -(lo.kw - 1 - j) * d, l, 1, l, 1.f), 0, lo.R, 0, lo.G, lo.p_dil_k[l] + (long long)j * lo.R * lo.G, lo.G);
+    if (lo.C > 0) append_wgrad_tiles(lt, proto(2, 0, 0, 1, l, 1.f), 0, lo.C, 0, lo.G, lo.p_c_k[l], lo.G);
     for (int m0 = 0; m0 < lo.Gh; m0 += 128) {
       if (l < lo.L - 1)
-        append_wgrad_tiles(lo.tiles_main, proto(3, 0, l, 4, l + 1, lo.res_scale), m0, 128, 0, lo.R, lo.p_o_k[l] + (long long)m0 * lo.R, lo.R);
-      append_wgrad_tiles(lo.tiles_main, proto(3, 0, l, 5, 0, lo.skip_scale[l]), m0, 128, 0, lo.S, lo.p_s_k[l] + (long long)m0 * lo.S, lo.S);
-    }
+        append_wgrad_tiles(lt, proto(3, 0, l, 4, l + 1, lo.res_scale), m0, 128, 0, lo.R, lo.p_o_k[l] + (long long)m0 * lo.R, lo.R);
+      append_wgrad_tiles(lt, proto(3, 0, l, 5, 0, lo.skip_scale[l]), m0, 128, 0, lo.S, lo.p_s_k[l] + (long long)m0 * lo.S, lo.S);
+    }
+    lo.tile_start[l] = int(lo.tiles_main.size());
+    const std::vector<WgradTile> slots = pair_wgrad_tiles(lt.data(), int(lt.size()));
+    lo.tiles_main.insert(lo.tiles_main.end(), slots.begin(), slots.end());
   }
   lo.tiles_head.clear();
   WgradTile f2 = proto(2, 0, 0, 3, 0, 1.f);
@@ -312,6 +316,8 @@
     for (int part = 0; part < (lo.mol ? 1 : 2); ++part)
       append_wgrad_tiles(lo.tiles_head, f2, m0, 128, part * 256, lo.O, lo.p_f2_k + (long long)m0 * lo.O, lo.O);
   }
+  lo.n_head_busy = int(lo.tiles_head.size());
+  lo.tiles_head = pair_wgrad_tiles(lo.tiles_head.data(), int(lo.tiles_head.size()));
   lo.n_tiles_main = int(lo.tiles_main.size());
   lo.tile_start[lo.L] = lo.n_tiles_main;
   lo.n_tiles_head = int(lo.tiles_head.size());
@@ -1297,6 +1303,16 @@
   return param_info(lo.params, i, name, name_cap, offset, ndim, shape4, nullptr);
 }
 
+extern "C" int t2_wn_wgrad_stats(const t2_wn_config_t* cfg, int which, long long* stats) {
+  Layout lo;
+  int rc = build_layout(cfg, lo);
+  if (rc) return rc;
+  T2_REQUIRE(stats && (which == 0 || which == 1), T2_ERR_INVALID_ARG, "wgrad_stats: bad arguments");
+  const std::vector<WgradTile>& t = which == 0 ? lo.tiles_main : lo.tiles_head;
+  wgrad_slot_stats(t.data(), int(t.size()), stats);
+  return T2_OK;
+}
+
 extern "C" int t2_wn_init(const t2_wn_config_t* cfg, void* d_packed, void* d_workspace, void* stream) {
   Layout lo;
   int rc = build_layout(cfg, lo);
@@ -1576,7 +1592,7 @@
   const ActT a_dg = make_act(dg, lo.G, lo.T, lo.B, lo.L);
   const int bn_z = lo.Gh >= 256 ? 256 : 128;
   if (use_chain(lo)) {
-    rc = launch_chain(lo, 1, ws, pk, d_params, 1, seed, d_step, side ? lo.n_tiles_head : 0, st);
+    rc = launch_chain(lo, 1, ws, pk, d_params, 1, seed, d_step, side ? lo.n_head_busy : 0, st);
     if (rc) return rc;
   } else {
     for (int l = lo.L - 1; l >= 0; --l) {
```
